# PaddlePaddle/Paddle3D

Hardware: NVIDIA H100
Metric: CenterPoint frames/sec @300k pts, 0.075m voxel (0.1m voxel: geometry_01m), 1440x1440x40 grid (higher is better)
Workload: dtype f16x3 (fp16 hi/lo' pairs, f32 accumulation)

## Files before the change

### include/p3d_b200.h

```cpp
#ifndef P3D_B200_H_
#define P3D_B200_H_

#include <stddef.h>
#include <stdint.h>

#ifdef __cplusplus
extern "C" {
#endif

typedef void *p3d_stream_t;

enum p3d_status {
  P3D_OK = 0,
  P3D_ERR_INVALID_ARG = -1,
  P3D_ERR_WORKSPACE = -2,
  P3D_ERR_CUDA = -3,
  P3D_ERR_UNSUPPORTED = -4
};

const char *p3d_status_string(int status);
int p3d_last_cuda_error(void);
int p3d_abi_version(void);

size_t p3d_hard_voxelize_workspace_bytes(int64_t num_points, int max_points, int max_voxels);
int p3d_hard_voxelize(const float *points, int64_t num_points, int num_point_dim, const float *voxel_size_host,
                      const float *point_cloud_range_host, int max_points, int max_voxels, float *voxels,
                      int32_t *coords, int32_t *num_points_per_voxel, int32_t *num_voxels, void *workspace,
                      size_t workspace_bytes, p3d_stream_t stream);

int p3d_voxelize_mean(const float *points, int64_t num_points, int num_point_dim, const float *voxel_size_host,
                      const float *point_cloud_range_host, int max_points, int max_voxels, int batch_id,
                      float *mean, int32_t *coors4, int32_t *num_points_per_voxel, int32_t *num_voxels,
                      void *workspace, size_t workspace_bytes, p3d_stream_t stream);

int p3d_voxel_mean(const float *voxels, const int32_t *num_points_per_voxel, const int32_t *num_voxels_dev,
                   int num_voxels_cap, int max_points, int num_point_dim, float *mean, p3d_stream_t stream);

size_t p3d_scatter_dense_workspace_bytes(int batch, int D, int ny, int nx);
int p3d_scatter_dense(const float *feats, const int32_t *coords, const int32_t *n_dev, int n_cap, int C,
                      int batch, int D, int ny, int nx, int use_z, float *out, void *workspace,
                      size_t workspace_bytes, p3d_stream_t stream);

int p3d_bev_pool_v2(const float *depth, const float *feat, const int32_t *ranks_depth, const int32_t *ranks_feat,
                    const int32_t *ranks_bev, const int32_t *interval_lengths, const int32_t *interval_starts,
                    int n_intervals, int c, float *out, int64_t out_numel, p3d_stream_t stream);
int p3d_bev_pool_v2_bkwd(const float *out_grad, const float *depth, const float *feat, const int32_t *ranks_depth,
                         const int32_t *ranks_feat, const int32_t *ranks_bev, const int32_t *interval_lengths,
                         const int32_t *interval_starts, int n_intervals, int c, float *depth_grad,
                         int64_t depth_numel, float *feat_grad, int64_t feat_numel, p3d_stream_t stream);

int p3d_boxes_overlap_bev(const float *boxes_a, int num_a, const float *boxes_b, int num_b, float *overlap,
                          p3d_stream_t stream);
int p3d_boxes_iou_bev(const float *boxes_a, int num_a, const float *boxes_b, int num_b, float *iou,
                      p3d_stream_t stream);
size_t p3d_nms_workspace_bytes(int n);
int p3d_nms(const float *boxes, int n, float nms_overlap_thresh, int normal, int32_t *keep, int32_t *num_keep,
            void *workspace, size_t workspace_bytes, p3d_stream_t stream);

size_t p3d_centerpoint_postprocess_workspace_bytes(int num_tasks, int feat_h, int feat_w, int nms_pre_max_size,
                                                    int nms_post_max_size);
int p3d_centerpoint_postprocess(int num_tasks, const float *const *hm, const int32_t *hm_channels_host,
                                const float *const *reg, const float *const *height, const float *const *dim,
                                const float *const *vel, const float *const *rot, int feat_h, int feat_w,
                                const float *voxel_size_host, const float *point_cloud_range_host,
                                const float *post_center_range_host, const int32_t *num_classes_host,
                                int down_ratio, float score_threshold, float nms_iou_threshold,
                                int nms_pre_max_size, int nms_post_max_size, int with_velocity, float *bboxes,
                                float *scores, int64_t *labels, int32_t *counts, void *workspace,
                                size_t workspace_bytes, p3d_stream_t stream);

size_t p3d_sparse_rulebook_workspace_bytes(int64_t n_in_cap, int64_t n_out_cap);
int p3d_sparse_rulebook_subm(const int32_t *coords, const int32_t *n_in_dev, int64_t n_in_cap, int batch,
                             const int *spatial_host, const int *ksize_host, int32_t *nbr, void *workspace,
                             size_t workspace_bytes, p3d_stream_t stream);
int p3d_sparse_rulebook_conv(const int32_t *coords, const int32_t *n_in_dev, int64_t n_in_cap, int batch,
                             const int *spatial_host, const int *ksize_host, const int *stride_host,
                             const int *pad_host, int32_t *out_coords, int32_t *n_out_dev, int64_t out_cap,
                             int32_t *nbr, void *workspace, size_t workspace_bytes, p3d_stream_t stream);

size_t p3d_sparse_table_bytes(int64_t rows_cap);
int p3d_sparse_table_build(const int32_t *coords, const int32_t *n_dev, int64_t n_cap, int batch,
                           const int *spatial_host, void *table, size_t table_bytes, p3d_stream_t stream);
int p3d_sparse_rulebook_subm_t(const int32_t *coords, const int32_t *n_dev, int64_t n_cap, int batch,
                               const int *spatial_host, const int *ksize_host, const void *table, size_t table_bytes,
                               int32_t *nbr, p3d_stream_t stream);
int p3d_sparse_rulebook_conv_t(const int32_t *coords, const int32_t *n_in_dev, int64_t n_in_cap, int batch,
                               const int *spatial_host, const int *ksize_host, const int *stride_host,
                               const int *pad_host, const void *table_in, size_t table_in_bytes, int32_t *out_coords,
                               int32_t *n_out_dev, int64_t out_cap, void *table_out, size_t table_out_bytes,
                               int32_t *nbr, p3d_stream_t stream);

int p3d_sparse_rulebook_level_t(const int32_t *coords, const int32_t *n_in_dev, int64_t n_in_cap, int batch,
                                const int *spatial_host, const int *ksize_host, const int *stride_host,
                                const int *pad_host, const void *table_in, size_t table_in_bytes, int32_t *out_coords,
                                int32_t *n_out_dev, int64_t out_cap, void *table_out, size_t table_out_bytes,
                                int32_t *nbr, const int *subm_ksize_host, int32_t *nbr_subm, p3d_stream_t stream);

int p3d_sparse_affine_act(const float *x, const int32_t *n_dev, int64_t n_cap, int C, const float *scale,
                          const float *shift, const float *residual, int relu, float *out, p3d_stream_t stream);

enum p3d_conv_precision { P3D_CONV_FP32 = 0, P3D_CONV_TF32X3 = 1 };
size_t p3d_sparse_conv_packed_weight_bytes(int K, int Cin, int Cout);
int p3d_sparse_conv_pack_weights(const float *weight, int K, int Cin, int Cout, float *packed, p3d_stream_t stream);
int p3d_sparse_conv_gather_gemm(const float *in, const int32_t *nbr, const int32_t *n_out_dev, int64_t n_out_cap,
                                int K, int Cin, int Cout, const float *weight, const float *scale,
                                const float *shift, const float *residual, int relu, int precision, float *out,
                                p3d_stream_t stream);

size_t p3d_sparse_conv_splitk_workspace_bytes(int64_t n_out_cap, int Cin, int Cout);
int p3d_sparse_conv_gather_gemm_tf32x3_ws(const float *in, const int32_t *nbr, const int32_t *n_out_dev,
                                          int64_t n_out_cap, int K, int Cin, int Cout, const float *packed_weight,
                                          const float *scale, const float *shift, const float *residual, int relu,
                                          float *out, void *workspace, size_t workspace_bytes, p3d_stream_t stream);

int p3d_rows_convert_layout(const float *src, int src_layout, const int32_t *n_dev, int64_t n_cap, int C, float *dst,
                            p3d_stream_t stream);
int p3d_sparse_conv_gather_gemm_split(const float *in_split, const int32_t *nbr, const int32_t *n_out_dev,
                                      int64_t n_out_cap, int K, int Cin, int Cout, const float *packed_weight,
                                      const float *scale, const float *shift, const float *residual_split, int relu,
                                      float *out_f32, float *out_split, p3d_stream_t stream);
int p3d_sparse_conv_gather_gemm_split_ws(const float *in_split, const int32_t *nbr, const int32_t *n_out_dev,
                                         int64_t n_out_cap, int K, int Cin, int Cout, const float *packed_weight,
                                         const float *scale, const float *shift, const float *residual_split, int relu,
                                         float *out_f32, float *out_split, void *workspace, size_t workspace_bytes,
                                         p3d_stream_t stream);
int p3d_sparse_conv_gather_gemm_split_tma(const float *in_split, int64_t n_in_rows, const int32_t *nbr,
                                          const int32_t *n_out_dev, int64_t n_out_cap, int K, int Cin, int Cout,
                                          const float *packed_weight, const float *scale, const float *shift,
                                          const float *residual_split, int relu, float *out_f32, float *out_split,
                                          void *workspace, size_t workspace_bytes, p3d_stream_t stream);

int p3d_sparse_conv_small_cin_h16(const float *in, const int32_t *nbr, const int32_t *n_out_dev, int64_t n_out_cap, int K,
                                  int Cin, int Cout, const float *weight, const float *scale, const float *shift, int relu,
                                  float *out_f32, void *out_h16, int32_t *status_dev, p3d_stream_t stream);
int p3d_sparse_rows_to_pixel_h16(const void *rows_h16, const int32_t *coords, const int32_t *n_dev, int n_cap, int C,
                                 int batch, int D, int ny, int nx, void *out_pixel_h16, p3d_stream_t stream);
size_t p3d_sparse_conv_f16_packed_weight_bytes(int K, int Cin, int Cout);
int p3d_sparse_conv_f16_pack_weights(const float *weight, int K, int Cin, int Cout, void *packed, int32_t *status_dev,
                                     p3d_stream_t stream);
int p3d_rows_convert_h16(const void *src, int to_h16, const int32_t *n_dev, int64_t n_cap, int C, void *dst,
                         int32_t *status_dev, p3d_stream_t stream);
size_t p3d_sparse_conv_f16_workspace_bytes(int64_t n_out_cap, int Cout, int max_splits);
int p3d_sparse_conv_f16(const void *in_h16, const int32_t *nbr, const int32_t *n_out_dev, int64_t n_out_cap, int K,
                        int Cin, int Cout, const void *packed_weight, const float *scale, const float *shift,
                        const void *residual_h16, int relu, float *out_f32, void *out_h16, void *workspace,
                        size_t workspace_bytes, int max_splits, int32_t *status_dev, p3d_stream_t stream);

size_t p3d_sparse_conv_wm_packed_weight_bytes(int K, int Cin, int Cout);
int p3d_sparse_conv_wm_pack_weights(const float *weight, int K, int Cin, int Cout, void *packed, int32_t *status_dev,
                                    p3d_stream_t stream);
size_t p3d_sparse_conv_wm_workspace_bytes(int64_t n_out_cap, int Cout);
int p3d_sparse_conv_wm(const void *in_h16, const int32_t *nbr, const int32_t *n_out_dev, int64_t n_out_cap, int K, int Cin,
                       int Cout, const void *packed_weight, const float *scale, const float *shift,
                       const void *residual_h16, int relu, float *out_f32, void *out_h16, void *workspace,
                       size_t workspace_bytes, int32_t *status_dev, p3d_stream_t stream);

int p3d_nchw_to_pixel_split(const float *in, int B, int C, int H, int W, float *out_split, p3d_stream_t stream);
size_t p3d_dense_conv2d_packed_weight_bytes(int taps, int Cin, int Cout, int n_tile);
int p3d_dense_conv2d_split(const float *in_split, int B, int H, int W, int Cin, const float *packed_weight, int Cout,
                           int n_tile, int kh, int kw, int stride, int pad, int up, const float *scale,
                           const float *shift, int relu, float *out_split, int out_C, int out_c0, float *out_nchw,
                           p3d_stream_t stream);

int p3d_head_final_conv(const float *in_split, int B, int H, int W, int in_C, int Cin, int groups, const float *weight,
                        const float *bias, const int32_t *plane0_host, const int32_t *cnt_host, int planes,
                        float *out_nchw, p3d_stream_t stream);
int p3d_head_final_conv_h16(const void *in_h16, int B, int H, int W, int in_C, int Cin, int groups, const float *weight,
                            const float *bias, const int32_t *plane0_host, const int32_t *cnt_host, int planes,
                            float *out_nchw, p3d_stream_t stream);

int p3d_nchw_to_pixel_h16(const float *in, int B, int C, int H, int W, void *out_h16, int32_t *status_dev,
                          p3d_stream_t stream);
int p3d_pixel_h16_to_nchw(const void *in_h16, int B, int C, int H, int W, float *out, p3d_stream_t stream);
size_t p3d_dense_conv2d_f16_packed_weight_bytes(int taps, int Cin, int Cout, int n_tile);
int p3d_dense_conv2d_f16_pack_weights(const float *weight_tci, int taps, int Cin, int n_tile, void *packed,
                                      int32_t *status_dev, p3d_stream_t stream);
size_t p3d_bev_pool_prepare_workspace_bytes(int64_t num_points);
int p3d_bev_pool_prepare(const float *coor, int B, int N, int D, int H, int W, const float *grid_lower_bound_host,
                         const float *grid_interval_host, const int32_t *grid_size_host, int32_t *ranks_bev,
                         int32_t *ranks_depth, int32_t *ranks_feat, int32_t *interval_starts, int32_t *interval_lengths,
                         int32_t *counts_dev, void *workspace, size_t workspace_bytes, p3d_stream_t stream);

int p3d_grouped_head_conv_f16(const void *in_h16, int B, int H, int W, int in_C, int Cin, int groups,
                              const void *packed_weight, const float *bias, const int32_t *plane0_dev,
                              const int32_t *cnt_dev, int planes, float *out_nchw, int32_t *status_dev, p3d_stream_t stream);
int p3d_head_out_conv_f16(const void *in_h16, int B, int H, int W, int in_C, int Cin, int groups, const void *packed_weight,
                          const float *bias, const int32_t *cin0_dev, const int32_t *plane0_dev, const int32_t *cnt_dev,
                          int planes, float *out_nchw, p3d_stream_t stream);
int p3d_dense_conv2d_f16(const void *in_h16, int B, int H, int W, int Cin, const void *packed_weight, int Cout, int n_tile,
                         int kh, int kw, int stride, int pad, int up, const float *scale, const float *shift, int relu,
                         void *out_h16, int out_C, int out_c0, float *out_nchw, int mode, int m_tiles,
                         int32_t *status_dev, p3d_stream_t stream);

int p3d_pillar_feature_net(const float *voxels, const int32_t *num_points_per_voxel, const int32_t *coors,
                           const int32_t *num_voxels_dev, int64_t n_cap, int max_points, int num_point_dim,
                           int out_channels, const float *weight, const float *bn_scale, const float *bn_shift,
                           const float *voxel_size_host, const float *point_cloud_range_host, float *out,
                           p3d_stream_t stream);

size_t p3d_anchor_head_postprocess_workspace_bytes(int num_anchors, int grid_nx, int grid_ny, int nms_pre_max_size);
int p3d_anchor_head_postprocess(const float *head, int feat_h, int feat_w, int anchors_per_loc, const float *anchors,
                                const int32_t *anchor_corners, const int32_t *coords, const int32_t *num_coords_dev,
                                int coords_cap, int grid_nx, int grid_ny, int anchor_area_threshold, float score_threshold,
                                float nms_iou_threshold, int nms_pre_max_size, int nms_post_max_size,
                                const float *post_center_range_host, float *boxes, float *scores, int64_t *labels,
                                int32_t *counts, uint8_t *anchor_mask, float *sorted_boxes, float *sorted_scores,
                                void *workspace, size_t workspace_bytes, p3d_stream_t stream);

#ifdef __cplusplus
}
#endif
#endif
```

### paddle3d_b200/_lib.py

```python
import ctypes as C
import os

_HERE = os.path.dirname(os.path.abspath(__file__))
LIB_PATH = os.path.join(_HERE, "libp3d_b200.so")
_lib = None

c_f32p = C.c_void_p
_i64 = C.c_int64
_int = C.c_int
_f = C.c_float
_sz = C.c_size_t
_vp = C.c_void_p

SIGNATURES = {
    "p3d_status_string": (C.c_char_p, [_int]),
    "p3d_last_cuda_error": (_int, []),
    "p3d_abi_version": (_int, []),
    "p3d_hard_voxelize_workspace_bytes": (_sz, [_i64, _int, _int]),
    "p3d_hard_voxelize": (_int, [_vp, _i64, _int, _vp, _vp, _int, _int, _vp, _vp, _vp, _vp, _vp, _sz, _vp]),
    "p3d_voxelize_mean": (_int, [_vp, _i64, _int, _vp, _vp, _int, _int, _int, _vp, _vp, _vp, _vp, _vp, _sz, _vp]),
    "p3d_voxel_mean": (_int, [_vp, _vp, _vp, _int, _int, _int, _vp, _vp]),
    "p3d_scatter_dense_workspace_bytes": (_sz, [_int, _int, _int, _int]),
    "p3d_scatter_dense": (_int, [_vp, _vp, _vp, _int, _int, _int, _int, _int, _int, _int, _vp, _vp, _sz, _vp]),
    "p3d_bev_pool_v2": (_int, [_vp, _vp, _vp, _vp, _vp, _vp, _vp, _int, _int, _vp, _i64, _vp]),
    "p3d_bev_pool_v2_bkwd": (_int, [_vp, _vp, _vp, _vp, _vp, _vp, _vp, _vp, _int, _int, _vp, _i64, _vp, _i64, _vp]),
    "p3d_boxes_overlap_bev": (_int, [_vp, _int, _vp, _int, _vp, _vp]),
    "p3d_boxes_iou_bev": (_int, [_vp, _int, _vp, _int, _vp, _vp]),
    "p3d_nms_workspace_bytes": (_sz, [_int]),
    "p3d_nms": (_int, [_vp, _int, _f, _int, _vp, _vp, _vp, _sz, _vp]),
    "p3d_centerpoint_postprocess_workspace_bytes": (_sz, [_int, _int, _int, _int, _int]),
    "p3d_centerpoint_postprocess": (_int, [_int, _vp, _vp, _vp, _vp, _vp, _vp, _vp, _int, _int, _vp, _vp, _vp, _vp,
                                           _int, _f, _f, _int, _int, _int, _vp, _vp, _vp, _vp, _vp, _sz, _vp]),
    "p3d_sparse_rulebook_workspace_bytes": (_sz, [_i64, _i64]),
    "p3d_sparse_rulebook_subm": (_int, [_vp, _vp, _i64, _int, _vp, _vp, _vp, _vp, _sz, _vp]),
    "p3d_sparse_rulebook_conv": (_int, [_vp, _vp, _i64, _int, _vp, _vp, _vp, _vp, _vp, _vp, _i64, _vp, _vp, _sz,
                                        _vp]),
    "p3d_sparse_table_bytes": (_sz, [_i64]),
    "p3d_sparse_table_build": (_int, [_vp, _vp, _i64, _int, _vp, _vp, _sz, _vp]),
    "p3d_sparse_rulebook_subm_t": (_int, [_vp, _vp, _i64, _int, _vp, _vp, _vp, _sz, _vp, _vp]),
    "p3d_sparse_rulebook_conv_t": (_int, [_vp, _vp, _i64, _int, _vp, _vp, _vp, _vp, _vp, _sz, _vp, _vp, _i64, _vp, _sz,
                                          _vp, _vp]),
    "p3d_sparse_rulebook_level_t": (_int, [_vp, _vp, _i64, _int, _vp, _vp, _vp, _vp, _vp, _sz, _vp, _vp, _i64, _vp, _sz,
                                           _vp, _vp, _vp, _vp]),
    "p3d_sparse_affine_act": (_int, [_vp, _vp, _i64, _int, _vp, _vp, _vp, _int, _vp, _vp]),
    "p3d_sparse_conv_packed_weight_bytes": (_sz, [_int, _int, _int]),
    "p3d_sparse_conv_pack_weights": (_int, [_vp, _int, _int, _int, _vp, _vp]),
    "p3d_rows_convert_layout": (_int, [_vp, _int, _vp, _i64, _int, _vp, _vp]),
    "p3d_sparse_conv_gather_gemm_split": (_int, [_vp, _vp, _vp, _i64, _int, _int, _int, _vp, _vp, _vp, _vp, _int, _vp,
                                                 _vp, _vp]),
    "p3d_sparse_conv_gather_gemm_split_ws": (_int, [_vp, _vp, _vp, _i64, _int, _int, _int, _vp, _vp, _vp, _vp, _int, _vp,
                                                    _vp, _vp, _sz, _vp]),
    "p3d_sparse_conv_gather_gemm_split_tma": (_int, [_vp, _i64, _vp, _vp, _i64, _int, _int, _int, _vp, _vp, _vp, _vp, _int,
                                                     _vp, _vp, _vp, _sz, _vp]),
    "p3d_sparse_conv_splitk_workspace_bytes": (_sz, [_i64, _int, _int]),
    "p3d_sparse_conv_small_cin_h16": (_int, [_vp, _vp, _vp, _i64, _int, _int, _int, _vp, _vp, _vp, _int, _vp, _vp, _vp, _vp]),
    "p3d_sparse_rows_to_pixel_h16": (_int, [_vp, _vp, _vp, _int, _int, _int, _int, _int, _int, _vp, _vp]),
    "p3d_sparse_conv_f16_packed_weight_bytes": (_sz, [_int, _int, _int]),
    "p3d_sparse_conv_f16_pack_weights": (_int, [_vp, _int, _int, _int, _vp, _vp, _vp]),
    "p3d_rows_convert_h16": (_int, [_vp, _int, _vp, _i64, _int, _vp, _vp, _vp]),
    "p3d_sparse_conv_f16_workspace_bytes": (_sz, [_i64, _int, _int]),
    "p3d_sparse_conv_f16": (_int, [_vp, _vp, _vp, _i64, _int, _int, _int, _vp, _vp, _vp, _vp, _int, _vp, _vp, _vp, _sz,
                                   _int, _vp, _vp]),
    "p3d_sparse_conv_wm_packed_weight_bytes": (_sz, [_int, _int, _int]),
    "p3d_sparse_conv_wm_pack_weights": (_int, [_vp, _int, _int, _int, _vp, _vp, _vp]),
    "p3d_sparse_conv_wm_workspace_bytes": (_sz, [_i64, _int]),
    "p3d_sparse_conv_wm": (_int, [_vp, _vp, _vp, _i64, _int, _int, _int, _vp, _vp, _vp, _vp, _int, _vp, _vp, _vp, _sz,
                                  _vp, _vp]),
    "p3d_nchw_to_pixel_split": (_int, [_vp, _int, _int, _int, _int, _vp, _vp]),
    "p3d_dense_conv2d_packed_weight_bytes": (_sz, [_int, _int, _int, _int]),
    "p3d_pillar_feature_net": (_int, [_vp, _vp, _vp, _vp, _i64, _int, _int, _int, _vp, _vp, _vp, _vp, _vp, _vp, _vp]),
    "p3d_head_final_conv": (_int, [_vp, _int, _int, _int, _int, _int, _int, _vp, _vp, _vp, _vp, _int, _vp, _vp]),
    "p3d_head_final_conv_h16": (_int, [_vp, _int, _int, _int, _int, _int, _int, _vp, _vp, _vp, _vp, _int, _vp, _vp]),
    "p3d_nchw_to_pixel_h16": (_int, [_vp, _int, _int, _int, _int, _vp, _vp, _vp]),
    "p3d_pixel_h16_to_nchw": (_int, [_vp, _int, _int, _int, _int, _vp, _vp]),
    "p3d_dense_conv2d_f16_packed_weight_bytes": (_sz, [_int, _int, _int, _int]),
    "p3d_dense_conv2d_f16_pack_weights": (_int, [_vp, _int, _int, _int, _vp, _vp, _vp]),
    "p3d_bev_pool_prepare_workspace_bytes": (_sz, [_i64]),
    "p3d_bev_pool_prepare": (_int, [_vp, _int, _int, _int, _int, _int, _vp, _vp, _vp, _vp, _vp, _vp, _vp, _vp, _vp, _vp, _sz,
                                    _vp]),
    "p3d_head_out_conv_f16": (_int, [_vp, _int, _int, _int, _int, _int, _int, _vp, _vp, _vp, _vp, _vp, _int, _vp, _vp]),
    "p3d_grouped_head_conv_f16": (_int, [_vp, _int, _int, _int, _int, _int, _int, _vp, _vp, _vp, _vp, _int, _vp, _vp, _vp]),
    "p3d_dense_conv2d_f16": (_int, [_vp, _int, _int, _int, _int, _vp, _int, _int, _int, _int, _int, _int, _int, _vp, _vp,
                                    _int, _vp, _int, _int, _vp, _int, _int, _vp, _vp]),
    "p3d_dense_conv2d_split": (_int, [_vp, _int, _int, _int, _int, _vp, _int, _int, _int, _int, _int, _int, _int, _vp, _vp,
                                      _int, _vp, _int, _int, _vp, _vp]),
    "p3d_sparse_conv_gather_gemm_tf32x3_ws": (_int, [_vp, _vp, _vp, _i64, _int, _int, _int, _vp, _vp, _vp, _vp, _int, _vp,
                                                     _vp, _sz, _vp]),
    "p3d_sparse_conv_gather_gemm": (_int, [_vp, _vp, _vp, _i64, _int, _int, _int, _vp, _vp, _vp, _vp, _int, _int,
                                           _vp, _vp]),
    "p3d_anchor_head_postprocess_workspace_bytes": (_sz, [_int, _int, _int, _int]),
    "p3d_anchor_head_postprocess": (_int, [_vp, _int, _int, _int, _vp, _vp, _vp, _vp, _int, _int, _int, _int, _f, _f,
                                           _int, _int, _vp, _vp, _vp, _vp, _vp, _vp, _vp, _vp, _vp, _sz, _vp]),
}


class P3DError(RuntimeError):
    pass


def lib():
    global _lib
    if _lib is None:
        if not os.path.exists(LIB_PATH):
            raise P3DError("libp3d_b200.so is not built: run `python -c 'import __graft_entry__ as g; g.build()'` "
                           "(paddle3d_b200 has no CPU or library fallback)")
        _lib = C.CDLL(LIB_PATH)
        for name, (res, args) in SIGNATURES.items():
            fn = getattr(_lib, name)
            fn.restype = res
            fn.argtypes = args
    return _lib


_DEBUG_SYNC = bool(os.environ.get("P3D_DEBUG_SYNC"))


def check(rc, what):
    if _DEBUG_SYNC and rc == 0:
        import torch
        try:
            torch.cuda.synchronize()
        except Exception as e:
            raise P3DError("%s: kernel fault (%s)" % (what, e))
    if rc != 0:
        l = lib()
        msg = l.p3d_status_string(rc).decode()
        extra = " (cudaError %d)" % l.p3d_last_cuda_error() if rc == -3 else ""
        raise P3DError("%s failed: %s%s" % (what, msg, extra))


def fptr(arr):
    return C.cast(arr, C.c_void_p)


def host_floats(vals):
    return (C.c_float * len(vals))(*[float(v) for v in vals])


def host_ints(vals):
    return (C.c_int * len(vals))(*[int(v) for v in vals])
```

### paddle3d_b200/csrc/dense_conv_f16.cu

```cuda
#include <cuda.h>
#include <cuda_fp16.h>

#include "p3d_b200.h"
#include "tc_common.cuh"

namespace p3d {
namespace dcf {

using namespace tc;

constexpr int kTW = 8, kTH = 16;
constexpr int kMaxA = 6, kMaxB = 12;
constexpr int kDenseThreads = 384;
constexpr uint32_t kConsumerWarps = 8;
constexpr uint32_t kEpiThreads = 96;
constexpr float kLoScale = 2048.0f, kLoInv = 1.0f / 2048.0f;

struct Params {
  int B, H, W, Cin;
  int taps, kw, stride, pad;
  int up;
  int oH, oW;
  int tiles_x, tiles_y, n_ntiles;
  int cout;
  int out_H, out_W;
  int out_C, out_c0;
  int relu;
  const uint8_t *packed_w;
  const float *scale, *shift;
  uint8_t *out_h16;
  float *out_nchw;
  int32_t *status;
  int grouped, in_C;
  const int32_t *grp_plane0, *grp_cnt;
  int base_offset_mode;
  int w_bytes;
};

template <int N, int MT, bool HALO, int PITCH, bool WS = false>
struct Cfg {
  static constexpr int A_ROWS = HALO ? PITCH * (kTH * MT + 2) : kM * MT;
  static constexpr int A_BYTES = ((A_ROWS * 128 + 1023) / 1024) * 1024;
  static constexpr int B_BYTES = 128 * N;
  static constexpr int B_BLK = 64 * N;
  static constexpr bool STAGE = !WS;
  static constexpr int SP = N + 8;
  static constexpr int STG_WG = MT * 64 * SP;
  static constexpr int STG_BYTES = STAGE ? 2 * STG_WG * 4 : 0;
  static constexpr int AVAIL = (227 - 6) * 1024 - STG_BYTES;
  static constexpr int NA_TAP_RAW = AVAIL / (A_BYTES + B_BYTES);
  static constexpr int NA = WS ? 3 : (HALO ? 2 : (NA_TAP_RAW > kMaxA ? kMaxA : NA_TAP_RAW));
  static constexpr int BUDGET = AVAIL - NA * A_BYTES;
  static constexpr int NB_RAW = BUDGET / B_BYTES;
  static constexpr int NB = NB_RAW > kMaxB ? kMaxB : NB_RAW;
  static constexpr int ACC = MT * N;
  static constexpr int SPU = HALO ? 9 : 1;
  static constexpr int P_REGS = STAGE ? 88 : 40, C_REGS = STAGE ? 208 : 232;
  static_assert(128 * P_REGS + 256 * C_REGS <= kDenseThreads * 168, "register split");
  static_assert(N == 16 || N == 64 || N == 128, "N tile: 16 (grouped output convs), 64 or 128");
  static_assert(MT == 1 || MT == 2, "one or two M tiles");
  static_assert(MT * N <= 128, "accumulators: at most 128 registers per thread");
  static_assert(WS || NB >= 3, "weight ring too shallow");
  static_assert(NA >= 2 && NA <= kMaxA, "activation ring depth");
  static_assert(!WS || (HALO && MT == 1), "weight-stationary: haloed 3x3 tiles, one M tile");
};

__device__ __forceinline__ void tma_tile4d(uint32_t dst, const CUtensorMap *map, int c, int x, int y, int b, uint32_t bar) {
  asm volatile(
      "cp.async.bulk.tensor.4d.shared::cluster.global.tile.mbarrier::complete_tx::bytes [%0], [%1, {%2, %3, %4, %5}], [%6];" ::
          "r"(dst),
      "l"(reinterpret_cast<uint64_t>(map)), "r"(c), "r"(x), "r"(y), "r"(b), "r"(bar)
      : "memory");
}
__device__ __forceinline__ void split_h16(float x, __half &hi, __half &lo, bool &ovf) {
  if (fabsf(x) > 65504.0f) {
    ovf = true;
    x = copysignf(65504.0f, x);
  }
  hi = __float2half_rn(x);
  lo = __float2half_rn((x - __half2float(hi)) * kLoScale);
}

__device__ __forceinline__ void split_h16x2(float a, float b, __half2 &hi, __half2 &lo, bool &ovf) {
  if (fabsf(a) > 65504.0f) {
    ovf = true;
    a = copysignf(65504.0f, a);
  }
  if (fabsf(b) > 65504.0f) {
    ovf = true;
    b = copysignf(65504.0f, b);
  }
  hi = __floats2half2_rn(a, b);
  const float2 h = __half22float2(hi);
  lo = __floats2half2_rn((a - h.x) * kLoScale, (b - h.y) * kLoScale);
}

struct Item {
  int nt, tap0, tx0, ty0, b;
};

enum TraceField {
  kTrItems, kTrCycles,
  kTrAFull, kTrBFull = kTrAFull + 2,
  kTrMma = kTrBFull + 2,
  kTrEpi = kTrMma + 2,
  kTrStageFree = kTrEpi + 2,
  kTrAEmpty = kTrStageFree + 2, kTrBEmpty,
  kTrEwWait, kTrEwBusy,
  kTrFields
};
#ifdef P3D_DENSE_TRACE
constexpr int kTrMaxCtas = 1024;
__device__ unsigned long long g_dense_trace[kTrMaxCtas][kTrFields];
struct Trace {
  unsigned long long sum[kTrFields] = {};
  __device__ __forceinline__ long long now() const { return clock64(); }
  __device__ __forceinline__ void add(int f, long long t0) { sum[f] += static_cast<unsigned long long>(clock64() - t0); }
  __device__ __forceinline__ void count(int f, unsigned long long v) { sum[f] += v; }
  __device__ void flush(int cw) const {
#pragma unroll
    for (int f = 0; f < kTrFields; ++f) {
      const int dst = f >= kTrAFull && f < kTrAEmpty ? f + cw : f;
      if (sum[f]) atomicAdd(&g_dense_trace[blockIdx.x % kTrMaxCtas][dst], sum[f]);
    }
  }
};
#else
struct Trace {
  __device__ __forceinline__ long long now() const { return 0; }
  __device__ __forceinline__ void add(int, long long) {}
  __device__ __forceinline__ void count(int, unsigned long long) {}
  __device__ __forceinline__ void flush(int) const {}
};
#endif
template <bool WS = false>
__device__ __forceinline__ Item decode(long long w, const Params &p, int th) {
  Item it;
  long long q = w;
  if (WS) {
    const long long pix = static_cast<long long>(p.B) * p.tiles_y * p.tiles_x;
    it.nt = static_cast<int>(q / pix);
    q -= it.nt * pix;
  } else {
    it.nt = static_cast<int>(q % p.n_ntiles);
    q /= p.n_ntiles;
  }
  it.tap0 = 0;
  if (p.up > 1) {
    const int up2 = p.up * p.up;
    it.tap0 = static_cast<int>(q % up2);
    q /= up2;
  }
  it.tx0 = static_cast<int>(q % p.tiles_x) * kTW;
  q /= p.tiles_x;
  it.ty0 = static_cast<int>(q % p.tiles_y) * th;
  it.b = static_cast<int>(q / p.tiles_y);
  return it;
}

template <int N, int MT>
__device__ __forceinline__ void epilogue_warps(const Params &p, const float *stg, unsigned long long *staged,
                                               unsigned long long *freed, long long n_items, long long w_first,
                                               long long w_step, int th, int et) {
  constexpr int SP = N + 8, ROWS = MT * 64;
  const int ew = et >> 5, lane = et & 31;
  bool ovf = false;
  Trace tr;
  for (long long idx = 0; idx < n_items; ++idx) {
    const Item im = decode<false>(w_first + idx * w_step, p, th);
    const int g_cnt = p.grouped ? __ldg(p.grp_cnt + im.nt) : 0, g_p0 = p.grouped ? __ldg(p.grp_plane0 + im.nt) : 0;
    const int dy = p.up > 1 ? im.tap0 / p.up : 0, dx = p.up > 1 ? im.tap0 % p.up : 0;
    for (int c = 0; c < 2; ++c) {
      long long t0 = tr.now();
      mbar_wait(smem_u32(staged + c), static_cast<uint32_t>(idx & 1));
      tr.add(kTrEwWait, t0);
      t0 = tr.now();
      const float *st = stg + c * ROWS * SP;
      auto pixel = [&](int r, int &Y, int &X) {
        const int m = c * 64 + (r & 63), iy = im.ty0 + (r >> 6) * kTH + m / kTW, ix = im.tx0 + m % kTW;
        Y = iy * p.up + dy;
        X = ix * p.up + dx;
        return iy < p.oH && ix < p.oW;
      };
      if (N >= 32 && p.out_h16) {
        const int r4 = lane >> 3, c4 = (lane & 7) * 4;
        for (int q = 0; q < N / 32; ++q) {
          const int col = q * 32 + c4, ch = im.nt * N + col, oc = p.out_c0 + ch;
          if (ch >= p.cout) continue;
          float sc[4], sh[4];
#pragma unroll
          for (int e = 0; e < 4; ++e) {
            sc[e] = p.scale ? __ldg(p.scale + ch + e) : 1.0f;
            sh[e] = p.shift ? __ldg(p.shift + ch + e) : 0.0f;
          }
#pragma unroll 2
          for (int rq = ew; rq < ROWS / 4; rq += 3) {
            const int r = rq * 4 + r4;
            int Y, X;
            if (!pixel(r, Y, X)) continue;
            const float4 o4 = *reinterpret_cast<const float4 *>(st + r * SP + col);
            float v[4] = {o4.x, o4.y, o4.z, o4.w};
#pragma unroll
            for (int e = 0; e < 4; ++e) {
              v[e] = fmaf(v[e], sc[e], sh[e]);
              if (p.relu) v[e] = fmaxf(v[e], 0.f);
            }
            __half2 h01, l01, h23, l23;
            split_h16x2(v[0], v[1], h01, l01, ovf);
            split_h16x2(v[2], v[3], h23, l23, ovf);
            uint8_t *op = p.out_h16 + ((static_cast<size_t>(im.b) * p.out_H + Y) * p.out_W + X) * (4 * static_cast<size_t>(p.out_C)) +
                          (oc / 32) * 128 + (oc % 32) * 2;
            *reinterpret_cast<uint2 *>(op) = make_uint2(*reinterpret_cast<const uint32_t *>(&h01), *reinterpret_cast<const uint32_t *>(&h23));
            *reinterpret_cast<uint2 *>(op + 64) = make_uint2(*reinterpret_cast<const uint32_t *>(&l01), *reinterpret_cast<const uint32_t *>(&l23));
          }
        }
      }
      if (p.out_nchw) {
        const int px = lane & 7, cc = lane >> 3;
        for (int u = ew; u < (ROWS / 8) * (N / 4); u += 3) {
          const int r = (u % (ROWS / 8)) * 8 + px, col = (u / (ROWS / 8)) * 4 + cc, ch = im.nt * N + col;
          int Y, X;
          if ((p.grouped ? col >= g_cnt : ch >= p.cout) || !pixel(r, Y, X)) continue;
          const float sc = p.scale ? __ldg(p.scale + ch) : 1.0f, sh = p.shift ? __ldg(p.shift + ch) : 0.0f;
          float v = fmaf(st[r * SP + col], sc, sh);
          if (p.relu) v = fmaxf(v, 0.f);
          const int plane = p.grouped ? g_p0 + col : ch;
          p.out_nchw[((static_cast<size_t>(im.b) * p.cout + plane) * p.out_H + Y) * p.out_W + X] = v;
        }
      }
      mbar_arrive(smem_u32(freed + c));
      tr.add(kTrEwBusy, t0);
    }
  }
  if (ovf && p.status) atomicOr(p.status, 1);
  if (et == 0) tr.flush(0);
}

template <int N, int MT, bool HALO, int PITCH, bool WS = false>
__global__ void __launch_bounds__(kDenseThreads, 1)
    dense_conv_f16_kernel(const __grid_constant__ CUtensorMap in_map, const Params p) {
  using C = Cfg<N, MT, HALO, PITCH, WS>;
  constexpr int TH = kTH * MT;
  constexpr int H = N / 2;
  asm volatile("griddepcontrol.launch_dependents;" ::: "memory");
  asm volatile("griddepcontrol.wait;" ::: "memory");
  const int up2 = p.up * p.up;
  const long long n_total = static_cast<long long>(p.B) * p.tiles_y * p.tiles_x * p.n_ntiles * (p.up > 1 ? up2 : 1);
  if (static_cast<long long>(blockIdx.x) >= n_total) return;
  const long long w_first = WS ? (static_cast<long long>(blockIdx.x) * n_total) / gridDim.x : blockIdx.x;
  const long long n_work = WS ? (static_cast<long long>(blockIdx.x + 1) * n_total) / gridDim.x : n_total;
  const long long w_step = WS ? 1 : gridDim.x;
  const long long n_items = (n_work - w_first + w_step - 1) / w_step;

  extern __shared__ __align__(1024) uint8_t smem_raw[];
  uint8_t *smem = reinterpret_cast<uint8_t *>((reinterpret_cast<uintptr_t>(smem_raw) + 1023) & ~uintptr_t(1023));
  __shared__ __align__(8) unsigned long long s_bar[2 * kMaxA + 2 * kMaxB + 6];
  constexpr int kAF = 0, kAE = kMaxA, kBF = 2 * kMaxA, kBE = 2 * kMaxA + kMaxB, kWF = 2 * kMaxA + 2 * kMaxB, kWE = kWF + 1;
  constexpr int kSS = kWE + 1, kSF = kSS + 2;

  const int tid = threadIdx.x, wg = tid >> 7, wtid = tid & 127;
  if (tid == 0) {
    for (int s = 0; s < C::NA; ++s) {
      mbar_init(smem_u32(&s_bar[kAF + s]), 1);
      mbar_init(smem_u32(&s_bar[kAE + s]), kConsumerWarps);
    }
    for (int s = 0; s < (WS ? 0 : C::NB); ++s) {
      mbar_init(smem_u32(&s_bar[kBF + s]), 1);
      mbar_init(smem_u32(&s_bar[kBE + s]), kConsumerWarps);
    }
    mbar_init(smem_u32(&s_bar[kWF]), 1);
    mbar_init(smem_u32(&s_bar[kWE]), kConsumerWarps);
    for (int c = 0; c < 2; ++c) {
      mbar_init(smem_u32(&s_bar[kSS + c]), 128);
      mbar_init(smem_u32(&s_bar[kSF + c]), kEpiThreads);
    }
    fence_mbar_init();
  }
  __syncthreads();
  const uint32_t a_ring = smem_u32(smem);
  const uint32_t b_ring = a_ring + C::NA * C::A_BYTES;
  float *const stg = reinterpret_cast<float *>(smem + C::NA * C::A_BYTES + C::NB * C::B_BYTES);
  const int G = p.Cin / 32;
  const int taps_item = p.up > 1 ? 1 : p.taps;
  const int units_item = HALO ? G : taps_item * G;
  auto item_w = [&](long long idx) { return w_first + idx * w_step; };

  if (wg == 0) {
    asm volatile("setmaxnreg.dec.sync.aligned.u32 %0;" ::"n"(C::P_REGS));
    if (tid >= 32) {
      if (C::STAGE) epilogue_warps<N, MT>(p, stg, s_bar + kSS, s_bar + kSF, n_items, w_first, w_step, TH, tid - 32);
      return;
    }
    if (tid != 0) return;
    uint32_t a_slot = 0, a_ph = 0, b_slot = 0, b_ph = 0;
    int cur_nt = -1;
    uint32_t img = 0;
    Trace tr;
    for (long long idx = 0; idx < n_items; ++idx) {
      const Item im = decode<WS>(item_w(idx), p, TH);
      const int cg0 = p.grouped ? im.nt * G : 0;
      const uint8_t *w_tile = p.packed_w + static_cast<size_t>(im.nt) * p.taps * (p.Cin / 16) * C::B_BLK;
      if (WS && im.nt != cur_nt) {
        if (img > 0) mbar_wait(smem_u32(&s_bar[kWE]), (img - 1) & 1u);
        const uint32_t bar = smem_u32(&s_bar[kWF]);
        mbar_arrive_expect_tx(bar, static_cast<uint32_t>(p.w_bytes));
        for (int off = 0; off < p.w_bytes; off += 16384) {
          const int bytes = p.w_bytes - off < 16384 ? p.w_bytes - off : 16384;
          bulk_g2s(b_ring + static_cast<uint32_t>(off), w_tile + off, static_cast<uint32_t>(bytes), bar);
        }
        ++img;
        cur_nt = im.nt;
      }
      int dy = 0, dx = 0;
      for (int tu = 0; tu < (HALO ? 1 : taps_item); ++tu) {
        const int tap = p.up > 1 ? im.tap0 : tu;
        for (int g = 0; g < G; ++g) {
          const uint32_t abar = smem_u32(&s_bar[kAF + a_slot]), a_dst = a_ring + a_slot * C::A_BYTES;
          const long long t0 = tr.now();
          mbar_wait(smem_u32(&s_bar[kAE + a_slot]), a_ph ^ 1u);
          tr.add(kTrAEmpty, t0);
          mbar_arrive_expect_tx(abar, static_cast<uint32_t>(C::A_ROWS * 128));
          if (HALO) {
            tma_tile4d(a_dst, &in_map, (cg0 + g) * 64, im.tx0 - 1, im.ty0 - 1, im.b, abar);
          } else {
            const int x = im.tx0 * p.stride - p.pad + dx, y = im.ty0 * p.stride - p.pad + dy;
            tma_tile4d(a_dst, &in_map, (cg0 + g) * 64, x, y, im.b, abar);
          }
          if (++a_slot == C::NA) a_slot = 0, a_ph ^= 1u;
          for (int t = 0; t < (WS ? 0 : C::SPU); ++t) {
            const uint32_t bbar = smem_u32(&s_bar[kBF + b_slot]);
            const long long t1 = tr.now();
            mbar_wait(smem_u32(&s_bar[kBE + b_slot]), b_ph ^ 1u);
            tr.add(kTrBEmpty, t1);
            mbar_arrive_expect_tx(bbar, static_cast<uint32_t>(C::B_BYTES));
            bulk_g2s(b_ring + b_slot * C::B_BYTES, w_tile + (static_cast<size_t>(HALO ? t : tap) * (p.Cin / 16) + 2 * g) * C::B_BLK,
                     static_cast<uint32_t>(C::B_BYTES), bbar);
            if (++b_slot == C::NB) b_slot = 0, b_ph ^= 1u;
          }
        }
        if (++dx == p.kw) dx = 0, ++dy;
      }
    }
    tr.flush(0);
    return;
  }

  asm volatile("setmaxnreg.inc.sync.aligned.u32 %0;" ::"n"(C::C_REGS));
  const int cw = wg - 1;
  const bool warp_leader = (tid & 31) == 0;
  auto release = [&](int base, uint32_t slot) {
    if (warp_leader) mbar_arrive(smem_u32(&s_bar[base + slot]));
  };
  bool ovf = false;
  uint32_t a_slot = 0, a_ph = 0, b_slot = 0, b_ph = 0;
  int cur_nt = -1;
  uint32_t img = 0;
  float acc[C::ACC];
  Trace tr;
  const long long t_start = tr.now();
  for (long long idx = 0; idx < n_items; ++idx) {
    const Item im = decode<WS>(item_w(idx), p, TH);
    if (WS && im.nt != cur_nt) {
      mbar_wait(smem_u32(&s_bar[kWF]), img & 1u);
      ++img;
      cur_nt = im.nt;
    }
#pragma unroll
    for (int i = 0; i < C::ACC; ++i) acc[i] = 0.f;
    uint32_t prev_b = 0;
    int prev_a = -1;
    bool pending = false;
    for (int ua = 0; ua < units_item; ++ua) {
      long long t0 = tr.now();
      mbar_wait(smem_u32(&s_bar[kAF + a_slot]), a_ph);
      tr.add(kTrAFull, t0);
      const uint32_t a_base = a_ring + a_slot * C::A_BYTES;
      for (int t = 0; t < C::SPU; ++t) {
        t0 = tr.now();
        if (!WS) mbar_wait(smem_u32(&s_bar[kBF + b_slot]), b_ph);
        tr.add(kTrBFull, t0);
        const uint32_t b_base = WS ? b_ring + static_cast<uint32_t>((t * (p.Cin / 16) + 2 * ua) * C::B_BLK)
                                   : b_ring + b_slot * C::B_BYTES;
        wg_fence();
#pragma unroll
        for (int kb = 0; kb < 2; ++kb) {
          const uint32_t bk = b_base + static_cast<uint32_t>(kb * C::B_BLK);
          const uint64_t dbh = smem_desc(bk, 2 * N * 16, 128), dbl = smem_desc(bk + N * 16, 2 * N * 16, 128);
#pragma unroll
          for (int mt = 0; mt < MT; ++mt) {
            uint32_t a0, sbo;
            if (HALO) {
              a0 = a_base + static_cast<uint32_t>(((mt * kTH + cw * 8 + t / 3) * PITCH + t % 3) * 128);
              sbo = PITCH * 128;
            } else {
              a0 = a_base + static_cast<uint32_t>((mt * kM + cw * 64) * 128);
              sbo = 1024;
            }
            const uint32_t ah = a0 + kb * 32, al = a0 + (2 + kb) * 32;
            const uint32_t bo = p.base_offset_mode ? 1u : 0u;
            const uint64_t dah = gmma_desc(ah, 16, sbo, 1, bo * ((ah >> 7) & 7u)), dal = gmma_desc(al, 16, sbo, 1, bo * ((al >> 7) & 7u));
            float *d = acc + mt * N;
            wg::mma_f16<N>(d, dah, dbh, 1u);
            wg::mma_f16<N>(d + H, dah, dbl, 1u);
            wg::mma_f16<N>(d + H, dal, dbh, 1u);
          }
        }
        wg_commit();
        t0 = tr.now();
        wg_wait<1>();
        tr.add(kTrMma, t0);
        if (pending) {
          if (!WS) release(kBE, prev_b);
          if (prev_a >= 0) release(kAE, static_cast<uint32_t>(prev_a));
        }
        pending = true;
        prev_b = b_slot;
        prev_a = t == C::SPU - 1 ? static_cast<int>(a_slot) : -1;
        if (!WS && ++b_slot == C::NB) b_slot = 0, b_ph ^= 1u;
      }
      if (++a_slot == C::NA) a_slot = 0, a_ph ^= 1u;
    }
    long long t0 = tr.now();
    wg_wait<0>();
    tr.add(kTrMma, t0);
    t0 = tr.now();
    if (!WS) release(kBE, prev_b);
    release(kAE, static_cast<uint32_t>(prev_a));
    if (WS && (idx + 1 == n_items || decode<WS>(item_w(idx + 1), p, TH).nt != im.nt)) release(kWE, 0);
    wg_fence_acc<C::ACC>(acc);
    if constexpr (C::STAGE) {
      tr.add(kTrEpi, t0);
      t0 = tr.now();
      if (idx > 0) mbar_wait(smem_u32(&s_bar[kSF + cw]), static_cast<uint32_t>((idx - 1) & 1));
      tr.add(kTrStageFree, t0);
      t0 = tr.now();
      float *const st = stg + cw * C::STG_WG;
#pragma unroll
      for (int mt = 0; mt < MT; ++mt) {
#pragma unroll
        for (int i = 0; i < H; i += 2) {
          const int r = mt * 64 + frag_row(i, wtid), c = frag_col(i, wtid);
          *reinterpret_cast<float2 *>(st + r * C::SP + c) =
              make_float2(fmaf(acc[mt * N + H + i], kLoInv, acc[mt * N + i]), fmaf(acc[mt * N + H + i + 1], kLoInv, acc[mt * N + i + 1]));
        }
      }
      mbar_arrive(smem_u32(&s_bar[kSS + cw]));
      tr.add(kTrEpi, t0);
      continue;
    }

    const int g_cnt = p.grouped ? __ldg(p.grp_cnt + im.nt) : 0, g_p0 = p.grouped ? __ldg(p.grp_plane0 + im.nt) : 0;
#pragma unroll
    for (int mt = 0; mt < MT; ++mt) {
#pragma unroll
      for (int i = 0; i < H; i += 2) {
        const int m = cw * 64 + frag_row(i, wtid), c = frag_col(i, wtid);
        const int iy = im.ty0 + mt * kTH + m / kTW, ix = im.tx0 + m % kTW;
        const int ch = im.nt * N + c;
        if (iy >= p.oH || ix >= p.oW || (p.grouped ? c >= g_cnt : ch >= p.cout)) continue;
        const int Y = iy * p.up + (p.up > 1 ? im.tap0 / p.up : 0), X = ix * p.up + (p.up > 1 ? im.tap0 % p.up : 0);
        const size_t opix = (static_cast<size_t>(im.b) * p.out_H + Y) * p.out_W + X;
        float v[2];
#pragma unroll
        for (int e = 0; e < 2; ++e) {
          const bool okc = p.grouped ? true : ch + e < p.cout;
          const float sc = (p.scale && okc) ? __ldg(p.scale + ch + e) : 1.0f, sh = (p.shift && okc) ? __ldg(p.shift + ch + e) : 0.0f;
          float o = fmaf(acc[mt * N + H + i + e], kLoInv, acc[mt * N + i + e]);
          o = fmaf(o, sc, sh);
          if (p.relu) o = fmaxf(o, 0.f);
          v[e] = o;
        }
        if (p.out_h16) {
          __half h0, l0, h1, l1;
          split_h16(v[0], h0, l0, ovf);
          split_h16(v[1], h1, l1, ovf);
          const int oc = p.out_c0 + ch;
          uint8_t *op = p.out_h16 + opix * (4 * static_cast<size_t>(p.out_C)) + (oc / 32) * 128 + (oc % 32) * 2;
          *reinterpret_cast<__half2 *>(op) = __halves2half2(h0, h1);
          *reinterpret_cast<__half2 *>(op + 64) = __halves2half2(l0, l1);
        }
        if (p.out_nchw) {
#pragma unroll
          for (int e = 0; e < 2; ++e) {
            if (p.grouped) {
              if (c + e < g_cnt) p.out_nchw[((static_cast<size_t>(im.b) * p.cout + g_p0 + c + e) * p.out_H + Y) * p.out_W + X] = v[e];
            } else if (ch + e < p.cout) {
              p.out_nchw[((static_cast<size_t>(im.b) * p.cout + ch + e) * p.out_H + Y) * p.out_W + X] = v[e];
            }
          }
        }
      }
    }
    tr.add(kTrEpi, t0);
  }
  if (ovf && p.status) atomicOr(p.status, 1);
  if (cw == 0) {
    tr.count(kTrItems, static_cast<unsigned long long>(n_items));
    tr.add(kTrCycles, t_start);
  }
  if (wtid == 0) tr.flush(cw);
}

__global__ void __launch_bounds__(256) nchw_to_pixel_h16_kernel(const float *__restrict__ in, int C, long long HW,
                                                                __half *__restrict__ out, int32_t *status) {
  __shared__ float s_t[32][33];
  const int b = blockIdx.z;
  const long long p0 = static_cast<long long>(blockIdx.x) * 32;
  const int c0 = blockIdx.y * 32;
  const int tx = threadIdx.x & 31, ty = threadIdx.x >> 5;
  for (int k = ty; k < 32; k += 8) {
    const int c = c0 + k;
    const long long px = p0 + tx;
    s_t[k][tx] = (c < C && px < HW) ? in[(static_cast<size_t>(b) * C + c) * HW + px] : 0.f;
  }
  __syncthreads();
  bool ovf = false;
  for (int k = ty; k < 32; k += 8) {
    const long long px = p0 + k;
    if (px < HW) {
      __half h, l;
      split_h16(s_t[tx][k], h, l, ovf);
      __half *grp = out + (static_cast<size_t>(b) * HW + px) * (2 * static_cast<size_t>(C)) + static_cast<size_t>(c0) * 2;
      grp[tx] = h;
      grp[32 + tx] = l;
    }
  }
  if (ovf && status) atomicOr(status, 1);
}

__global__ void __launch_bounds__(256) pixel_h16_to_nchw_kernel(const __half *__restrict__ in, int C, long long HW,
                                                                float *__restrict__ out, long long total) {
  const long long q = static_cast<long long>(blockIdx.x) * blockDim.x + threadIdx.x;
  if (q >= total) return;
  const long long px = q % HW;
  const int c = static_cast<int>((q / HW) % C);
  const long long b = q / (HW * C);
  const __half *grp = in + (b * HW + px) * (2 * static_cast<long long>(C)) + (c / 32) * 64;
  out[q] = fmaf(__half2float(grp[32 + c % 32]), kLoInv, __half2float(grp[c % 32]));
}

inline int make_image_map(const void *img, int B, int H, int W, int Cin, int stride, int box_x, int box_y, CUtensorMap *map) {
  using Encode = CUresult (*)(CUtensorMap *, CUtensorMapDataType, cuuint32_t, void *, const cuuint64_t *, const cuuint64_t *,
                              const cuuint32_t *, const cuuint32_t *, CUtensorMapInterleave, CUtensorMapSwizzle,
                              CUtensorMapL2promotion, CUtensorMapFloatOOBfill);
  static Encode encode = nullptr;
  if (!encode) {
    void *fn = nullptr;
    cudaDriverEntryPointQueryResult qr;
    if (cudaGetDriverEntryPoint("cuTensorMapEncodeTiled", &fn, cudaEnableDefault, &qr) != cudaSuccess || !fn)
      return P3D_ERR_UNSUPPORTED;
    encode = reinterpret_cast<Encode>(fn);
  }
  const cuuint64_t row = static_cast<cuuint64_t>(4) * Cin;
  const cuuint64_t gdim[4] = {static_cast<cuuint64_t>(2 * Cin), static_cast<cuuint64_t>(W), static_cast<cuuint64_t>(H),
                              static_cast<cuuint64_t>(B)};
  const cuuint64_t gstride[3] = {row, row * W, row * W * H};
  const cuuint32_t box[4] = {64u, static_cast<cuuint32_t>(box_x * stride), static_cast<cuuint32_t>(box_y * stride), 1u};
  const cuuint32_t estride[4] = {1u, static_cast<cuuint32_t>(stride), static_cast<cuuint32_t>(stride), 1u};
  const CUresult r = encode(map, CU_TENSOR_MAP_DATA_TYPE_FLOAT16, 4, const_cast<void *>(img), gdim, gstride, box, estride,
                            CU_TENSOR_MAP_INTERLEAVE_NONE, CU_TENSOR_MAP_SWIZZLE_128B, CU_TENSOR_MAP_L2_PROMOTION_NONE,
                            CU_TENSOR_MAP_FLOAT_OOB_FILL_NONE);
  return r == CUDA_SUCCESS ? P3D_OK : P3D_ERR_INVALID_ARG;
}

template <int N, int MT, bool HALO, int PITCH, bool WS = false>
int launch(const CUtensorMap &map, const Params &p, cudaStream_t st) {
  using C = Cfg<N, MT, HALO, PITCH, WS>;
  const size_t smem = static_cast<size_t>(C::NA) * C::A_BYTES +
                      (WS ? static_cast<size_t>(p.w_bytes) : static_cast<size_t>(C::NB) * C::B_BYTES) + C::STG_BYTES + 1024;
  if (smem > static_cast<size_t>(227 - 6) * 1024) return P3D_ERR_UNSUPPORTED;
  auto kern = dense_conv_f16_kernel<N, MT, HALO, PITCH, WS>;
  P3D_CUDA_CHECK(cudaFuncSetAttribute(kern, cudaFuncAttributeMaxDynamicSharedMemorySize, static_cast<int>(smem)));
  const long long work = static_cast<long long>(p.B) * p.tiles_y * p.tiles_x * p.n_ntiles * (p.up > 1 ? p.up * p.up : 1);
  cudaLaunchConfig_t cfg = {};
  const long long sms = num_sms();
  cfg.gridDim = dim3(static_cast<unsigned int>(work < sms ? work : sms));
  cfg.blockDim = dim3(kDenseThreads);
  cfg.dynamicSmemBytes = smem;
  cfg.stream = st;
  cudaLaunchAttribute attr[1];
  attr[0].id = cudaLaunchAttributeProgrammaticStreamSerialization;
  attr[0].val.programmaticStreamSerializationAllowed = 1;
  cfg.attrs = attr;
  cfg.numAttrs = 1;
  P3D_CUDA_CHECK(cudaLaunchKernelEx(&cfg, kern, map, p));
  P3D_LAUNCH_CHECK();
  return P3D_OK;
}

namespace out9 {
constexpr int kHT = 16, kOT = 14;
constexpr int kRows = kHT * kHT;
constexpr int kABytes = kRows * 128;
constexpr int kN = 32, kStride = 29;
constexpr int kWBlk = 64 * kN;
constexpr int kPBytes = kRows * kStride * 4;
constexpr int kMaxNA = 5, kNW = 3;
constexpr int kAcc = 2 * kN;

struct Params {
  int B, H, W, G;
  int tiles_x, tiles_y, groups, planes, NA;
  const uint8_t *packed_w;
  const float *bias;
  const int32_t *cin0;
  const int32_t *plane0, *cnt;
  float *out;
};

__global__ void __launch_bounds__(kThreads, 1) head_out9_kernel(const __grid_constant__ CUtensorMap in_map, const Params p) {
  asm volatile("griddepcontrol.launch_dependents;" ::: "memory");
  asm volatile("griddepcontrol.wait;" ::: "memory");
  const long long n_work = static_cast<long long>(p.B) * p.tiles_y * p.tiles_x * p.groups;
  if (static_cast<long long>(blockIdx.x) >= n_work) return;
  extern __shared__ __align__(1024) uint8_t smem_raw[];
  uint8_t *smem = reinterpret_cast<uint8_t *>((reinterpret_cast<uintptr_t>(smem_raw) + 1023) & ~uintptr_t(1023));
  __shared__ __align__(8) unsigned long long s_bar[kMaxNA + kNW];
  constexpr int kAF = 0, kWF = kMaxNA;
  const int tid = threadIdx.x, wg = tid >> 7, wtid = tid & 127;
  const int NA = p.NA, G = p.G;
  const uint32_t w_slot = static_cast<uint32_t>(2 * G * kWBlk);
  if (tid == 0) {
    for (int s = 0; s < NA; ++s) mbar_init(smem_u32(&s_bar[kAF + s]), 1);
    for (int s = 0; s < kNW; ++s) mbar_init(smem_u32(&s_bar[kWF + s]), 1);
    fence_mbar_init();
  }
  const uint32_t a_ring = smem_u32(smem);
  const uint32_t w_ring = a_ring + static_cast<uint32_t>(NA * kABytes);
  float *s_p = reinterpret_cast<float *>(smem + static_cast<size_t>(NA) * kABytes + static_cast<size_t>(kNW) * w_slot);

  auto decode = [&](long long w, int &g, int &tx0, int &ty0, int &b) {
    g = static_cast<int>(w % p.groups);
    long long q = w / p.groups;
    tx0 = static_cast<int>(q % p.tiles_x) * kOT;
    q /= p.tiles_x;
    ty0 = static_cast<int>(q % p.tiles_y) * kOT;
    b = static_cast<int>(q / p.tiles_y);
  };
  const long long n_items = (n_work - blockIdx.x + gridDim.x - 1) / gridDim.x;
  const long long n_steps = n_items * G;
  auto issue_a = [&](long long q) {
    int g, tx0, ty0, b;
    decode(blockIdx.x + (q / G) * gridDim.x, g, tx0, ty0, b);
    const int cg0 = (p.cin0 ? __ldg(p.cin0 + g) : g * G * 32) / 32;
    const uint32_t slot = static_cast<uint32_t>(q % NA), bar = smem_u32(&s_bar[kAF + slot]);
    mbar_arrive_expect_tx(bar, static_cast<uint32_t>(kABytes));
    tma_tile4d(a_ring + slot * kABytes, &in_map, (cg0 + static_cast<int>(q % G)) * 64, tx0 - 1, ty0 - 1, b, bar);
  };
  auto issue_w = [&](long long i) {
    const int g = static_cast<int>((blockIdx.x + i * gridDim.x) % p.groups);
    const uint32_t slot = static_cast<uint32_t>(i % kNW), bar = smem_u32(&s_bar[kWF + slot]);
    mbar_arrive_expect_tx(bar, w_slot);
    bulk_g2s(w_ring + slot * w_slot, p.packed_w + static_cast<size_t>(g) * w_slot, w_slot, bar);
  };

  long long next_a = 0, next_w = 0, q = 0;
  float acc[kAcc];
  for (long long idx = 0; idx < n_items; ++idx) {
    int g, tx0, ty0, b;
    decode(blockIdx.x + idx * gridDim.x, g, tx0, ty0, b);
    const int cnt = __ldg(p.cnt + g), p0 = __ldg(p.plane0 + g);
    const float4 bias = __ldg(reinterpret_cast<const float4 *>(p.bias) + g);
#pragma unroll
    for (int i = 0; i < kAcc; ++i) acc[i] = 0.f;
    const uint32_t ws = static_cast<uint32_t>(idx % kNW);
    for (int k = 0; k < G; ++k, ++q) {
      __syncthreads();
      if (tid == 0) {
        for (; next_a < n_steps && next_a <= q + NA - 1; ++next_a) issue_a(next_a);
        for (; next_w < n_items && (next_w - kNW + 1) * G <= q; ++next_w) issue_w(next_w);
      }
      if (k == 0) mbar_wait(smem_u32(&s_bar[kWF + ws]), static_cast<uint32_t>((idx / kNW) & 1));
      const uint32_t sa = static_cast<uint32_t>(q % NA);
      mbar_wait(smem_u32(&s_bar[kAF + sa]), static_cast<uint32_t>((q / NA) & 1));
      const uint32_t a_base = a_ring + sa * kABytes;
      const uint32_t w_base = w_ring + ws * w_slot;
      wg_fence();
#pragma unroll
      for (int kb = 0; kb < 2; ++kb) {
        const uint32_t bk = w_base + static_cast<uint32_t>((k * 2 + kb) * kWBlk);
        const uint64_t dbh = smem_desc(bk, 2 * kN * 16, 128), dbl = smem_desc(bk + kN * 16, 2 * kN * 16, 128);
#pragma unroll
        for (int mt = 0; mt < 2; ++mt) {
          const uint32_t a0 = a_base + static_cast<uint32_t>((mt * kM + wg * 64) * 128);
          const uint64_t dah = desc_sw128(a0 + kb * 32), dal = desc_sw128(a0 + (2 + kb) * 32);
          float *d = acc + mt * kN;
          wg::mma_f16<kN>(d, dah, dbh, 1u);
          wg::mma_f16<kN>(d + kN / 2, dah, dbl, 1u);
          wg::mma_f16<kN>(d + kN / 2, dal, dbh, 1u);
        }
      }
      wg_commit();
      wg_wait<0>();
    }
    wg_fence_acc<kAcc>(acc);
#pragma unroll
    for (int mt = 0; mt < 2; ++mt) {
#pragma unroll
      for (int i = 0; i < kN / 2; ++i) {
        const int r = mt * kM + wg * 64 + frag_row(i, wtid), c = frag_col(i, wtid);
        if (c < 27) s_p[r * kStride + c] = fmaf(acc[mt * kN + kN / 2 + i], kLoInv, acc[mt * kN + i]);
      }
    }
    __syncthreads();
    for (int o = tid; o < kOT * kOT; o += kThreads) {
      const int oy = o / kOT, ox = o - oy * kOT;
      const int Y = ty0 + oy, X = tx0 + ox;
      if (Y < p.H && X < p.W) {
        float s0 = bias.x, s1 = bias.y, s2 = bias.z;
#pragma unroll
        for (int t = 0; t < 9; ++t) {
          const float *e = s_p + ((oy + t / 3) * kHT + ox + t % 3) * kStride + t * 3;
          s0 += e[0];
          s1 += e[1];
          s2 += e[2];
        }
        float *op = p.out + ((static_cast<size_t>(b) * p.planes + p0) * p.H + Y) * p.W + X;
        const size_t plane = static_cast<size_t>(p.H) * p.W;
        op[0] = s0;
        if (cnt > 1) op[plane] = s1;
        if (cnt > 2) op[2 * plane] = s2;
      }
    }
  }
}
}

}
}

using namespace p3d;

extern "C" int p3d_nchw_to_pixel_h16(const float *in, int B, int C, int H, int W, void *out_h16, int32_t *status_dev,
                                     p3d_stream_t stream) {
  if (!in || !out_h16 || B < 1 || C < 32 || C % 32 || H < 1 || W < 1) return P3D_ERR_INVALID_ARG;
  const long long hw = static_cast<long long>(H) * W;
  dim3 grid(static_cast<unsigned int>((hw + 31) / 32), static_cast<unsigned int>(C / 32), B);
  dcf::nchw_to_pixel_h16_kernel<<<grid, 256, 0, static_cast<cudaStream_t>(stream)>>>(in, C, hw, static_cast<__half *>(out_h16),
                                                                                      status_dev);
  P3D_LAUNCH_CHECK();
  return P3D_OK;
}

extern "C" int p3d_pixel_h16_to_nchw(const void *in_h16, int B, int C, int H, int W, float *out, p3d_stream_t stream) {
  if (!in_h16 || !out || B < 1 || C < 32 || C % 32 || H < 1 || W < 1) return P3D_ERR_INVALID_ARG;
  const long long hw = static_cast<long long>(H) * W, total = hw * C * B;
  dcf::pixel_h16_to_nchw_kernel<<<div_up(total, 256), 256, 0, static_cast<cudaStream_t>(stream)>>>(
      static_cast<const __half *>(in_h16), C, hw, out, total);
  P3D_LAUNCH_CHECK();
  return P3D_OK;
}

#ifdef P3D_DENSE_TRACE
extern "C" int p3d_dense_trace_read(unsigned long long *host, int max_ctas, int reset) {
  const size_t n = static_cast<size_t>(max_ctas < dcf::kTrMaxCtas ? max_ctas : dcf::kTrMaxCtas) * dcf::kTrFields;
  P3D_CUDA_CHECK(cudaDeviceSynchronize());
  if (host) P3D_CUDA_CHECK(cudaMemcpyFromSymbol(host, dcf::g_dense_trace, n * sizeof(unsigned long long)));
  if (reset) {
    void *dev = nullptr;
    P3D_CUDA_CHECK(cudaGetSymbolAddress(&dev, dcf::g_dense_trace));
    P3D_CUDA_CHECK(cudaMemset(dev, 0, sizeof(dcf::g_dense_trace)));
    P3D_CUDA_CHECK(cudaDeviceSynchronize());
  }
  return dcf::kTrFields;
}
#endif

extern "C" size_t p3d_dense_conv2d_f16_packed_weight_bytes(int taps, int Cin, int Cout, int n_tile) {
  if (taps < 1 || Cin < 32 || Cin % 32 || Cout < 1 || (n_tile != 16 && n_tile != 32 && n_tile != 64 && n_tile != 128)) return 0;
  const size_t tiles = static_cast<size_t>((Cout + n_tile - 1) / n_tile);
  return align_up(tiles * taps * Cin * static_cast<size_t>(n_tile) * 4);
}

static int dense_conv_f16(const void *in_h16, int B, int H, int W, int Cin, const void *packed_weight, int Cout, int n_tile,
                          int kh, int kw, int stride, int pad, int up, const float *scale, const float *shift, int relu,
                          void *out_h16, int out_C, int out_c0, float *out_nchw, int mode, int m_tiles, int32_t *status_dev,
                          p3d_stream_t stream, int groups, int in_C, const int32_t *grp_plane0, const int32_t *grp_cnt) {
  if (!in_h16 || !packed_weight || (!out_h16 && !out_nchw) || B < 1 || H < 1 || W < 1 || Cout < 1) return P3D_ERR_INVALID_ARG;
  if (Cin < 32 || Cin % 32 || (n_tile != 64 && n_tile != 128 && !(groups && n_tile == 16))) return P3D_ERR_UNSUPPORTED;
  if (up < 1 || (up > 1 && (kh != up || kw != up || stride != up || pad != 0))) return P3D_ERR_UNSUPPORTED;
  if (up == 1 && (kh < 1 || kw < 1 || kh * kw > 32 || stride < 1 || stride > 2 || pad < 0)) return P3D_ERR_UNSUPPORTED;
  if (out_h16 && (Cout % 16 || out_C % 32 || out_c0 % 16 || out_c0 + Cout > out_C)) return P3D_ERR_INVALID_ARG;
  if ((reinterpret_cast<uintptr_t>(in_h16) & 15) || (reinterpret_cast<uintptr_t>(packed_weight) & 15) ||
      (reinterpret_cast<uintptr_t>(out_h16) & 15))
    return P3D_ERR_INVALID_ARG;
  dcf::Params p;
  p.B = B;
  p.H = H;
  p.W = W;
  p.Cin = Cin;
  p.taps = kh * kw;
  p.kw = kw;
  p.up = up;
  p.stride = up > 1 ? 1 : stride;
  p.pad = up > 1 ? 0 : pad;
  p.oH = up > 1 ? H : (H + 2 * pad - kh) / stride + 1;
  p.oW = up > 1 ? W : (W + 2 * pad - kw) / stride + 1;
  if (p.oH < 1 || p.oW < 1) return P3D_ERR_INVALID_ARG;
  p.out_H = up > 1 ? H * up : p.oH;
  p.out_W = up > 1 ? W * up : p.oW;
  p.n_ntiles = groups ? groups : (Cout + n_tile - 1) / n_tile;
  p.cout = Cout;
  p.grouped = groups ? 1 : 0;
  p.in_C = groups ? in_C : Cin;
  p.grp_plane0 = grp_plane0;
  p.grp_cnt = grp_cnt;
  p.out_C = out_C;
  p.out_c0 = out_c0;
  p.relu = relu;
  p.packed_w = static_cast<const uint8_t *>(packed_weight);
  p.scale = scale;
  p.shift = shift;
  p.out_h16 = static_cast<uint8_t *>(out_h16);
  p.out_nchw = out_nchw;
  p.status = status_dev;
  static const int env_mode = getenv("P3D_DENSE_MODE") ? atoi(getenv("P3D_DENSE_MODE")) : -1;
  static const int env_mt = getenv("P3D_DENSE_MT") ? atoi(getenv("P3D_DENSE_MT")) : -1;
  static const int env_pitch = getenv("P3D_DENSE_PITCH") ? atoi(getenv("P3D_DENSE_PITCH")) : 10;
  static const int env_bo = getenv("P3D_DENSE_BO") ? atoi(getenv("P3D_DENSE_BO")) : 0;
  p.base_offset_mode = env_bo;
  int pitch = env_pitch == 16 ? 16 : 10;
  if (env_mode >= 0) mode = env_mode;
  if (env_mt >= 0) m_tiles = env_mt;
  const bool halo = (mode == 0 || mode == 2) && up == 1 && kh == 3 && kw == 3 && stride == 1 && pad == 1;
  int mt = m_tiles;
  if (mt != 1 && mt != 2) {
    const long long tx = (p.oW + dcf::kTW - 1) / dcf::kTW, sms = num_sms();
    const long long per_row = static_cast<long long>(B) * tx * p.n_ntiles * (up > 1 ? up * up : 1);
    const long long items1 = per_row * ((p.oH + dcf::kTH - 1) / dcf::kTH), items2 = per_row * ((p.oH + 2 * dcf::kTH - 1) / (2 * dcf::kTH));
    mt = (n_tile <= 64 && 2 * ((items2 + sms - 1) / sms) <= (items1 + sms - 1) / sms) ? 2 : 1;
  }
  static const int env_ws = getenv("P3D_DENSE_WS") ? atoi(getenv("P3D_DENSE_WS")) : 0;
  p.w_bytes = p.taps * (Cin / 16) * 64 * n_tile;
  bool ws = false;
  if (halo && n_tile == 64 && !groups && pitch == 10 && (env_ws || mode == 2)) {
    const size_t need = 3 * static_cast<size_t>(dcf::Cfg<64, 1, true, 10, true>::A_BYTES) + p.w_bytes + 1024;
    const long long pix = static_cast<long long>(B) * ((p.oW + dcf::kTW - 1) / dcf::kTW) * ((p.oH + dcf::kTH - 1) / dcf::kTH);
    const long long items = pix * p.n_ntiles;
    ws = need <= static_cast<size_t>(227 - 6) * 1024 && (mode == 2 || items >= 8ll * num_sms());
  }
  if (mode == 2 && !ws) return P3D_ERR_UNSUPPORTED;
  if (ws || n_tile > 64) mt = 1;
  if (mt == 2) pitch = 10;
  p.tiles_x = (p.oW + dcf::kTW - 1) / dcf::kTW;
  p.tiles_y = (p.oH + dcf::kTH * mt - 1) / (dcf::kTH * mt);
  CUtensorMap map;
  const int bx = halo ? pitch : dcf::kTW, by = halo ? dcf::kTH * mt + 2 : dcf::kTH * mt;
  const int rc = dcf::make_image_map(in_h16, B, H, W, p.in_C, p.stride, bx, by, &map);
  if (rc != P3D_OK) return rc;
  cudaStream_t st = static_cast<cudaStream_t>(stream);
  if (ws) return dcf::launch<64, 1, true, 10, true>(map, p, st);
#define P3D_DCF(NT, M)                                                                          \
  if (n_tile == NT && mt == M) {                                                                \
    if (!halo) return dcf::launch<NT, M, false, 10>(map, p, st);                                \
    if (M == 1 && pitch == 16) return dcf::launch<NT, 1, true, 16>(map, p, st);                 \
    return dcf::launch<NT, M, true, 10>(map, p, st);                                            \
  }
  P3D_DCF(16, 1)
  P3D_DCF(16, 2)
  P3D_DCF(64, 1)
  P3D_DCF(64, 2)
  P3D_DCF(128, 1)
#undef P3D_DCF
  return P3D_ERR_UNSUPPORTED;
}

extern "C" int p3d_dense_conv2d_f16(const void *in_h16, int B, int H, int W, int Cin, const void *packed_weight, int Cout,
                                    int n_tile, int kh, int kw, int stride, int pad, int up, const float *scale,
                                    const float *shift, int relu, void *out_h16, int out_C, int out_c0, float *out_nchw,
                                    int mode, int m_tiles, int32_t *status_dev, p3d_stream_t stream) {
  return dense_conv_f16(in_h16, B, H, W, Cin, packed_weight, Cout, n_tile, kh, kw, stride, pad, up, scale, shift, relu, out_h16,
                        out_C, out_c0, out_nchw, mode, m_tiles, status_dev, stream, 0, 0, nullptr, nullptr);
}

extern "C" int p3d_grouped_head_conv_f16(const void *in_h16, int B, int H, int W, int in_C, int Cin, int groups,
                                         const void *packed_weight, const float *bias, const int32_t *plane0_dev,
                                         const int32_t *cnt_dev, int planes, float *out_nchw, int32_t *status_dev,
                                         p3d_stream_t stream) {
  if (!plane0_dev || !cnt_dev || groups < 1 || groups * Cin > in_C || in_C % 32 || planes < 1) return P3D_ERR_INVALID_ARG;
  return dense_conv_f16(in_h16, B, H, W, Cin, packed_weight, planes, 16, 3, 3, 1, 1, 1, nullptr, bias, 0, nullptr, 32, 0, out_nchw,
                        0, 0, status_dev, stream, groups, in_C, plane0_dev, cnt_dev);
}

extern "C" int p3d_head_out_conv_f16(const void *in_h16, int B, int H, int W, int in_C, int Cin, int groups,
                                     const void *packed_weight, const float *bias, const int32_t *cin0_dev,
                                     const int32_t *plane0_dev, const int32_t *cnt_dev, int planes, float *out_nchw,
                                     p3d_stream_t stream) {
  if (!in_h16 || !packed_weight || !bias || !plane0_dev || !cnt_dev || !out_nchw || B < 1 || H < 1 || W < 1 || groups < 1 ||
      planes < 1 || in_C % 32 || Cin > in_C)
    return P3D_ERR_INVALID_ARG;
  if (Cin != 32 && Cin != 64 && Cin != 128) return P3D_ERR_UNSUPPORTED;
  if ((reinterpret_cast<uintptr_t>(in_h16) & 15) || (reinterpret_cast<uintptr_t>(packed_weight) & 15) ||
      (reinterpret_cast<uintptr_t>(bias) & 15))
    return P3D_ERR_INVALID_ARG;
  namespace o9 = dcf::out9;
  o9::Params p;
  p.B = B;
  p.H = H;
  p.W = W;
  p.G = Cin / 32;
  p.tiles_x = (W + o9::kOT - 1) / o9::kOT;
  p.tiles_y = (H + o9::kOT - 1) / o9::kOT;
  p.groups = groups;
  p.planes = planes;
  p.NA = p.G <= 2 ? 5 : 4;
  p.packed_w = static_cast<const uint8_t *>(packed_weight);
  p.bias = bias;
  p.cin0 = cin0_dev;
  p.plane0 = plane0_dev;
  p.cnt = cnt_dev;
  p.out = out_nchw;
  CUtensorMap map;
  const int rc = dcf::make_image_map(in_h16, B, H, W, in_C, 1, o9::kHT, o9::kHT, &map);
  if (rc != P3D_OK) return rc;
  const size_t smem = static_cast<size_t>(p.NA) * o9::kABytes + static_cast<size_t>(o9::kNW) * 2 * p.G * o9::kWBlk + o9::kPBytes + 1024;
  auto kern = o9::head_out9_kernel;
  P3D_CUDA_CHECK(cudaFuncSetAttribute(kern, cudaFuncAttributeMaxDynamicSharedMemorySize, static_cast<int>(smem)));
  const long long work = static_cast<long long>(B) * p.tiles_y * p.tiles_x * groups;
  cudaLaunchConfig_t cfg = {};
  const long long sms = num_sms();
  cfg.gridDim = dim3(static_cast<unsigned int>(work < sms ? work : sms));
  cfg.blockDim = dim3(tc::kThreads);
  cfg.dynamicSmemBytes = smem;
  cfg.stream = static_cast<cudaStream_t>(stream);
  cudaLaunchAttribute attr[1];
  attr[0].id = cudaLaunchAttributeProgrammaticStreamSerialization;
  attr[0].val.programmaticStreamSerializationAllowed = 1;
  cfg.attrs = attr;
  cfg.numAttrs = 1;
  P3D_CUDA_CHECK(cudaLaunchKernelEx(&cfg, kern, map, p));
  P3D_LAUNCH_CHECK();
  return P3D_OK;
}
```

### paddle3d_b200/ops/dense_conv.py

```python
import torch

from .._lib import check, lib
from .._mem import ptr, require_cuda, stream


def n_tile_for(cout):
    return 128 if cout >= 128 else (64 if cout > 16 else 16)


def nchw_to_pixel_split(x):
    x = require_cuda(x, "x", torch.float32)
    b, c, h, w = x.shape
    out = torch.empty((b * h * w, 2 * c), dtype=torch.float32, device=x.device)
    check(lib().p3d_nchw_to_pixel_split(ptr(x), b, c, h, w, ptr(out), stream(x.device)), "nchw_to_pixel_split")
    return out


def _pack(w_tci, n_tile):
    L = lib()
    taps, cin, cout = w_tci.shape
    tiles = (cout + n_tile - 1) // n_tile
    total = L.p3d_dense_conv2d_packed_weight_bytes(taps, cin, cout, n_tile)
    if not total:
        raise ValueError("unsupported dense conv shape: taps %d Cin %d Cout %d" % (taps, cin, cout))
    packed = torch.zeros((total // 4,), dtype=torch.float32, device=w_tci.device)
    padded = torch.zeros((taps, cin, tiles * n_tile), dtype=torch.float32, device=w_tci.device)
    padded[:, :, :cout] = w_tci
    block = taps * cin * 2 * n_tile
    for t in range(tiles):
        wt = padded[:, :, t * n_tile:(t + 1) * n_tile].contiguous()
        dst = packed[t * block:(t + 1) * block]
        check(L.p3d_sparse_conv_pack_weights(ptr(wt), taps, cin, n_tile, ptr(dst), stream(wt.device)),
              "sparse_conv_pack_weights")
    return packed


def pack_conv_weight(weight, n_tile):
    weight = require_cuda(weight, "weight", torch.float32)
    cout, cin, kh, kw = weight.shape
    return _pack(weight.permute(2, 3, 1, 0).reshape(kh * kw, cin, cout).contiguous(), n_tile)


def pack_deconv_weight(weight, n_tile):
    weight = require_cuda(weight, "weight", torch.float32)
    cin, cout, k, k2 = weight.shape
    return _pack(weight.permute(2, 3, 0, 1).reshape(k * k2, cin, cout).contiguous(), n_tile)


def dense_conv2d(x_split, shape, packed, cout, n_tile, kernel, stride=1, padding=0, up=1, scale=None, shift=None,
                 relu=False, out_split=None, out_channels=None, out_c0=0, want_nchw=False):
    x_split = require_cuda(x_split, "x_split", torch.float32)
    b, h, w, cin = [int(v) for v in shape]
    if up > 1:
        oh, ow = h * up, w * up
        kh = kw = st = up
        pd = 0
    else:
        kh = kw = int(kernel)
        st, pd = int(stride), int(padding)
        oh, ow = (h + 2 * pd - kh) // st + 1, (w + 2 * pd - kw) // st + 1
    dev = x_split.device
    oc = int(out_channels or cout)
    if out_split is None and not want_nchw:
        out_split = torch.empty((b * oh * ow, 2 * oc), dtype=torch.float32, device=dev)
    out_nchw = torch.empty((b, cout, oh, ow), dtype=torch.float32, device=dev) if want_nchw else None
    check(lib().p3d_dense_conv2d_split(ptr(x_split), b, h, w, cin, ptr(packed), int(cout), int(n_tile), kh, kw, st, pd,
                                       int(up), ptr(scale), ptr(shift), int(relu), ptr(out_split), oc, int(out_c0),
                                       ptr(out_nchw), stream(dev)), "dense_conv2d_split")
    return out_split, out_nchw, (b, oh, ow)


def n_tile_for_f16(cout, cin=None, kernel=None, stride=1, padding=0, up=1):
    import os
    forced = os.environ.get("P3D_DENSE_NTILE")
    if forced and cout >= 128:
        return int(forced)
    if (cin is not None and kernel == 3 and stride == 1 and padding == 1 and up == 1 and cin <= 64 and cout >= 256
            and os.environ.get("P3D_DENSE_WS", "0") != "0"):
        return 64
    return 128 if cout >= 128 else 64


def _status(dev):
    from . import sparse_nn as sp
    return sp.status_tensor(dev)


def nchw_to_pixel_h16(x):
    x = require_cuda(x, "x", torch.float32)
    b, c, h, w = x.shape
    out = torch.empty((b * h * w, 2 * c), dtype=torch.float16, device=x.device)
    check(lib().p3d_nchw_to_pixel_h16(ptr(x), b, c, h, w, ptr(out), ptr(_status(x.device)), stream(x.device)),
          "nchw_to_pixel_h16")
    return out


def pixel_h16_to_nchw(x_h16, shape):
    b, h, w, c = [int(v) for v in shape]
    out = torch.empty((b, c, h, w), dtype=torch.float32, device=x_h16.device)
    check(lib().p3d_pixel_h16_to_nchw(ptr(x_h16), b, c, h, w, ptr(out), stream(x_h16.device)), "pixel_h16_to_nchw")
    return out


def _pack_f16(w_tci, n_tile):
    L = lib()
    taps, cin, cout = w_tci.shape
    tiles = (cout + n_tile - 1) // n_tile
    total = L.p3d_dense_conv2d_f16_packed_weight_bytes(taps, cin, cout, n_tile)
    if not total:
        raise ValueError("unsupported dense conv shape: taps %d Cin %d Cout %d" % (taps, cin, cout))
    packed = torch.zeros((total,), dtype=torch.uint8, device=w_tci.device)
    padded = torch.zeros((taps, cin, tiles * n_tile), dtype=torch.float32, device=w_tci.device)
    padded[:, :, :cout] = w_tci
    block = taps * cin * n_tile * 4
    for t in range(tiles):
        wt = padded[:, :, t * n_tile:(t + 1) * n_tile].contiguous()
        dst = packed[t * block:(t + 1) * block]
        check(L.p3d_dense_conv2d_f16_pack_weights(ptr(wt), taps, cin, n_tile, ptr(dst), ptr(_status(wt.device)),
                                                  stream(wt.device)), "dense_conv2d_f16_pack_weights")
    return packed


def pack_conv_weight_f16(weight, n_tile):
    weight = require_cuda(weight, "weight", torch.float32)
    cout, cin, kh, kw = weight.shape
    return _pack_f16(weight.permute(2, 3, 1, 0).reshape(kh * kw, cin, cout).contiguous(), n_tile)


def pack_deconv_weight_f16(weight, n_tile):
    weight = require_cuda(weight, "weight", torch.float32)
    cin, cout, k, k2 = weight.shape
    return _pack_f16(weight.permute(2, 3, 0, 1).reshape(k * k2, cin, cout).contiguous(), n_tile)


def dense_conv2d_f16(x_h16, shape, packed, cout, n_tile, kernel, stride=1, padding=0, up=1, scale=None, shift=None,
                     relu=False, out_h16=None, out_channels=None, out_c0=0, want_nchw=False, mode=0, m_tiles=0):
    x_h16 = require_cuda(x_h16, "x_h16", torch.float16)
    b, h, w, cin = [int(v) for v in shape]
    if up > 1:
        oh, ow = h * up, w * up
        kh = kw = st = up
        pd = 0
    else:
        kh = kw = int(kernel)
        st, pd = int(stride), int(padding)
        oh, ow = (h + 2 * pd - kh) // st + 1, (w + 2 * pd - kw) // st + 1
    dev = x_h16.device
    oc = int(out_channels or cout)
    if out_h16 is None and not want_nchw:
        out_h16 = torch.empty((b * oh * ow, 2 * oc), dtype=torch.float16, device=dev)
    out_nchw = torch.empty((b, cout, oh, ow), dtype=torch.float32, device=dev) if want_nchw else None
    check(lib().p3d_dense_conv2d_f16(ptr(x_h16), b, h, w, cin, ptr(packed), int(cout), int(n_tile), kh, kw, st, pd, int(up),
                                     ptr(scale), ptr(shift), int(relu), ptr(out_h16), oc, int(out_c0), ptr(out_nchw),
                                     int(mode), int(m_tiles), ptr(_status(dev)), stream(dev)), "dense_conv2d_f16")
    return out_h16, out_nchw, (b, oh, ow)
```

### paddle_ext/p3d_paddle_ops.cc

```cpp
#include <vector>

#include "paddle/extension.h"
#include "p3d_b200.h"

#define P3D_CHECK_GPU(x) PD_CHECK((x).is_gpu() || (x).is_gpu_pinned(), #x " must be a GPU Tensor.")
#define P3D_CALL(expr)                                                                 \
  do {                                                                                 \
    int _rc = (expr);                                                                  \
    if (_rc != 0) PD_THROW(std::string(#expr " failed: ") + p3d_status_string(_rc)); \
  } while (0)

namespace {

paddle::Tensor workspace(size_t bytes) {
  return paddle::empty({static_cast<int64_t>(bytes ? bytes : 256)}, paddle::DataType::UINT8, paddle::GPUPlace());
}

}

std::vector<paddle::Tensor> hard_voxelize(const paddle::Tensor &points, const std::vector<float> &voxel_size,
                                          const std::vector<float> &point_cloud_range,
                                          const int max_num_points_in_voxel, const int max_voxels) {
  P3D_CHECK_GPU(points);
  const int64_t n = points.shape()[0];
  const int f = static_cast<int>(points.shape()[1]);
  auto voxels = paddle::empty({max_voxels, max_num_points_in_voxel, f}, paddle::DataType::FLOAT32, paddle::GPUPlace());
  auto coords = paddle::empty({max_voxels, 3}, paddle::DataType::INT32, paddle::GPUPlace());
  auto npv = paddle::empty({max_voxels}, paddle::DataType::INT32, paddle::GPUPlace());
  auto num_voxels = paddle::empty({1}, paddle::DataType::INT32, paddle::GPUPlace());
  const size_t ws_bytes = p3d_hard_voxelize_workspace_bytes(n, max_num_points_in_voxel, max_voxels);
  auto ws = workspace(ws_bytes);
  P3D_CALL(p3d_hard_voxelize(points.data<float>(), n, f, voxel_size.data(), point_cloud_range.data(),
                             max_num_points_in_voxel, max_voxels, voxels.data<float>(), coords.data<int>(),
                             npv.data<int>(), num_voxels.data<int>(), ws.data<uint8_t>(), ws_bytes, points.stream()));
  return {voxels, coords, npv, num_voxels};
}

std::vector<std::vector<int64_t>> HardInferShape(std::vector<int64_t> points_shape, const std::vector<float> &voxel_size,
                                                 const std::vector<float> &point_cloud_range,
                                                 const int &max_num_points_in_voxel, const int &max_voxels) {
  return {{max_voxels, max_num_points_in_voxel, points_shape[1]}, {max_voxels, 3}, {max_voxels}, {1}};
}

std::vector<paddle::DataType> HardInferDtype(paddle::DataType points_dtype) {
  return {points_dtype, paddle::DataType::INT32, paddle::DataType::INT32, paddle::DataType::INT32};
}

PD_BUILD_OP(hard_voxelize)
    .Inputs({"POINTS"})
    .Outputs({"VOXELS", "COORS", "NUM_POINTS_PER_VOXEL", "num_voxels"})
    .SetKernelFn(PD_KERNEL(hard_voxelize))
    .Attrs({"voxel_size: std::vector<float>", "point_cloud_range: std::vector<float>", "max_num_points_in_voxel: int",
            "max_voxels: int"})
    .SetInferShapeFn(PD_INFER_SHAPE(HardInferShape))
    .SetInferDtypeFn(PD_INFER_DTYPE(HardInferDtype));

static std::vector<paddle::Tensor> pairwise(const paddle::Tensor &a, const paddle::Tensor &b, bool iou) {
  P3D_CHECK_GPU(a);
  P3D_CHECK_GPU(b);
  const int na = static_cast<int>(a.shape()[0]), nb = static_cast<int>(b.shape()[0]);
  auto out = paddle::empty({na, nb}, paddle::DataType::FLOAT32, paddle::GPUPlace());
  if (iou)
    P3D_CALL(p3d_boxes_iou_bev(a.data<float>(), na, b.data<float>(), nb, out.data<float>(), a.stream()));
  else
    P3D_CALL(p3d_boxes_overlap_bev(a.data<float>(), na, b.data<float>(), nb, out.data<float>(), a.stream()));
  return {out};
}
std::vector<paddle::Tensor> boxes_iou_bev_gpu(const paddle::Tensor &a, const paddle::Tensor &b) { return pairwise(a, b, true); }
std::vector<paddle::Tensor> boxes_overlap_bev_gpu(const paddle::Tensor &a, const paddle::Tensor &b) {
  return pairwise(a, b, false);
}

static std::vector<paddle::Tensor> nms_any(const paddle::Tensor &boxes, float thresh, int normal) {
  P3D_CHECK_GPU(boxes);
  const int n = static_cast<int>(boxes.shape()[0]);
  auto keep_dev = paddle::empty({n > 0 ? n : 1}, paddle::DataType::INT32, paddle::GPUPlace());
  auto num_dev = paddle::empty({1}, paddle::DataType::INT32, paddle::GPUPlace());
  const size_t ws_bytes = p3d_nms_workspace_bytes(n);
  auto ws = workspace(ws_bytes);
  P3D_CALL(p3d_nms(boxes.data<float>(), n, thresh, normal, keep_dev.data<int>(), num_dev.data<int>(),
                   ws.data<uint8_t>(), ws_bytes, boxes.stream()));
  return {keep_dev.copy_to(paddle::CPUPlace(), true), num_dev.copy_to(paddle::CPUPlace(), true)};
}
std::vector<paddle::Tensor> nms_gpu(const paddle::Tensor &boxes, float nms_overlap_thresh) {
  return nms_any(boxes, nms_overlap_thresh, 0);
}
std::vector<paddle::Tensor> nms_normal_gpu(const paddle::Tensor &boxes, float nms_overlap_thresh) {
  return nms_any(boxes, nms_overlap_thresh, 1);
}

std::vector<paddle::DataType> PairInferDtype(paddle::DataType a, paddle::DataType b) { return {a}; }
std::vector<std::vector<int64_t>> PairInferShape(std::vector<int64_t> a, std::vector<int64_t> b) { return {{a[0], b[0]}}; }
std::vector<paddle::DataType> NmsInferDtype(paddle::DataType boxes_dtype) {
  return {paddle::DataType::INT64, paddle::DataType::INT64};
}
std::vector<std::vector<int64_t>> NmsInferShape(std::vector<int64_t> boxes_shape) { return {{boxes_shape[0]}, {1}}; }

PD_BUILD_OP(boxes_iou_bev_gpu)
    .Inputs({"boxes_a_tensor", " boxes_b_tensor"})
    .Outputs({"ans_iou_tensor"})
    .SetKernelFn(PD_KERNEL(boxes_iou_bev_gpu))
    .SetInferDtypeFn(PD_INFER_DTYPE(PairInferDtype))
    .SetInferShapeFn(PD_INFER_SHAPE(PairInferShape));
PD_BUILD_OP(boxes_overlap_bev_gpu)
    .Inputs({"boxes_a", " boxes_b"})
    .Outputs({"ans_overlap"})
    .SetKernelFn(PD_KERNEL(boxes_overlap_bev_gpu))
    .SetInferDtypeFn(PD_INFER_DTYPE(PairInferDtype))
    .SetInferShapeFn(PD_INFER_SHAPE(PairInferShape));
PD_BUILD_OP(nms_gpu)
    .Inputs({"boxes"})
    .Outputs({"keep", "num_to_keep"})
    .Attrs({"nms_overlap_thresh: float"})
    .SetKernelFn(PD_KERNEL(nms_gpu))
    .SetInferDtypeFn(PD_INFER_DTYPE(NmsInferDtype))
    .SetInferShapeFn(PD_INFER_SHAPE(NmsInferShape));
PD_BUILD_OP(nms_normal_gpu)
    .Inputs({"boxes"})
    .Outputs({"keep", "num_to_keep"})
    .Attrs({"nms_overlap_thresh: float"})
    .SetKernelFn(PD_KERNEL(nms_normal_gpu))
    .SetInferDtypeFn(PD_INFER_DTYPE(NmsInferDtype))
    .SetInferShapeFn(PD_INFER_SHAPE(NmsInferShape));

std::vector<paddle::Tensor> centerpoint_postprocess(
    const std::vector<paddle::Tensor> &hm, const std::vector<paddle::Tensor> &reg,
    const std::vector<paddle::Tensor> &height, const std::vector<paddle::Tensor> &dim,
    const std::vector<paddle::Tensor> &vel, const std::vector<paddle::Tensor> &rot, const std::vector<float> &voxel_size,
    const std::vector<float> &point_cloud_range, const std::vector<float> &post_center_range,
    const std::vector<int> &num_classes, const int down_ratio, const float score_threshold,
    const float nms_iou_threshold, const int nms_pre_max_size, const int nms_post_max_size, const bool with_velocity) {
  if (!hm[0].is_gpu()) PD_THROW("Unsupported device type for centerpoint postprocess operator.");
  PD_CHECK(hm[0].shape()[0] == 1, "hm[0] batch size must be 1.");
  const int T = static_cast<int>(hm.size());
  const int H = static_cast<int>(hm[0].shape()[2]), W = static_cast<int>(hm[0].shape()[3]);
  std::vector<const float *> p[6];
  std::vector<int32_t> hm_c(T);
  const std::vector<paddle::Tensor> *lists[6] = {&hm, &reg, &height, &dim, &vel, &rot};
  for (int k = 0; k < 6; ++k)
    for (int t = 0; t < T; ++t) p[k].push_back((*lists[k])[t].data<float>());
  for (int t = 0; t < T; ++t) hm_c[t] = static_cast<int32_t>(hm[t].shape()[1]);
  const int dims = with_velocity ? 9 : 7;
  const int rows = T * (nms_post_max_size > 1 ? nms_post_max_size : 1);
  auto bboxes = paddle::empty({rows, dims}, paddle::DataType::FLOAT32, paddle::GPUPlace());
  auto scores = paddle::empty({rows}, paddle::DataType::FLOAT32, paddle::GPUPlace());
  auto labels = paddle::empty({rows}, paddle::DataType::INT64, paddle::GPUPlace());
  auto counts = paddle::empty({T + 1}, paddle::DataType::INT32, paddle::GPUPlace());
  const size_t ws_bytes = p3d_centerpoint_postprocess_workspace_bytes(T, H, W, nms_pre_max_size, nms_post_max_size);
  auto ws = workspace(ws_bytes);
  P3D_CALL(p3d_centerpoint_postprocess(T, p[0].data(), hm_c.data(), p[1].data(), p[2].data(), p[3].data(), p[4].data(),
                                       p[5].data(), H, W, voxel_size.data(), point_cloud_range.data(),
                                       post_center_range.data(), num_classes.data(), down_ratio, score_threshold,
                                       nms_iou_threshold, nms_pre_max_size, nms_post_max_size, with_velocity ? 1 : 0,
                                       bboxes.data<float>(), scores.data<float>(), labels.data<int64_t>(),
                                       counts.data<int>(), ws.data<uint8_t>(), ws_bytes, hm[0].stream()));
  const int k = counts.copy_to(paddle::CPUPlace(), true).data<int>()[T];
  return {paddle::experimental::slice(bboxes, {0}, {0}, {k}, {}, {}), paddle::experimental::slice(scores, {0}, {0}, {k}, {}, {}),
          paddle::experimental::slice(labels, {0}, {0}, {k}, {}, {})};
}

std::vector<std::vector<int64_t>> PostProcessInferShape(
    const std::vector<std::vector<int64_t>> &hm_shape, const std::vector<std::vector<int64_t>> &reg_shape,
    const std::vector<std::vector<int64_t>> &height_shape, const std::vector<std::vector<int64_t>> &dim_shape,
    const std::vector<std::vector<int64_t>> &vel_shape, const std::vector<std::vector<int64_t>> &rot_shape,
    const std::vector<float> &voxel_size, const std::vector<float> &point_cloud_range,
    const std::vector<float> &post_center_range, const std::vector<int> &num_classes, const int down_ratio,
    const float score_threshold, const float nms_iou_threshold, const int nms_pre_max_size,
    const int nms_post_max_size, const bool with_velocity) {
  if (with_velocity) return {{-1, 9}, {-1}, {-1}};
  return {{-1, 7}, {-1}, {-1}};
}

std::vector<paddle::DataType> PostProcessInferDtype(
    const std::vector<paddle::DataType> &hm_dtype, const std::vector<paddle::DataType> &reg_dtype,
    const std::vector<paddle::DataType> &height_dtype, const std::vector<paddle::DataType> &dim_dtype,
    const std::vector<paddle::DataType> &vel_dtype, const std::vector<paddle::DataType> &rot_dtype) {
  return {reg_dtype[0], hm_dtype[0], paddle::DataType::INT64};
}

PD_BUILD_OP(centerpoint_postprocess)
    .Inputs({paddle::Vec("HM"), paddle::Vec("REG"), paddle::Vec("HEIGHT"), paddle::Vec("DIM"), paddle::Vec("VEL"),
             paddle::Vec("ROT")})
    .Outputs({"BBOXES", "SCORES", "LABELS"})
    .SetKernelFn(PD_KERNEL(centerpoint_postprocess))
    .Attrs({"voxel_size: std::vector<float>", "point_cloud_range: std::vector<float>",
            "post_center_range: std::vector<float>", "num_classes: std::vector<int>", "down_ratio: int",
            "score_threshold: float", "nms_iou_threshold: float", "nms_pre_max_size: int", "nms_post_max_size: int",
            "with_velocity: bool"})
    .SetInferShapeFn(PD_INFER_SHAPE(PostProcessInferShape))
    .SetInferDtypeFn(PD_INFER_DTYPE(PostProcessInferDtype));

std::vector<paddle::Tensor> bev_pool_v2_forward(const paddle::Tensor &_depth, const paddle::Tensor &_feat,
                                                const paddle::Tensor &_ranks_depth, const paddle::Tensor &_ranks_feat,
                                                const paddle::Tensor &_ranks_bev, const paddle::Tensor &_interval_lengths,
                                                const paddle::Tensor &_interval_starts,
                                                const std::vector<int> &_bev_feat_shape) {
  P3D_CHECK_GPU(_feat);
  const int c = static_cast<int>(_feat.shape()[3]);
  const int n_intervals = static_cast<int>(_interval_lengths.shape()[0]);
  std::vector<int64_t> shape(_bev_feat_shape.begin(), _bev_feat_shape.end());
  auto out = paddle::empty(shape, _feat.type(), paddle::GPUPlace());
  P3D_CALL(p3d_bev_pool_v2(_depth.data<float>(), _feat.data<float>(), _ranks_depth.data<int>(), _ranks_feat.data<int>(),
                           _ranks_bev.data<int>(), _interval_lengths.data<int>(), _interval_starts.data<int>(),
                           n_intervals, c, out.data<float>(), out.numel(), _feat.stream()));
  return {out};
}

std::vector<paddle::Tensor> bev_pool_v2_backward(const paddle::Tensor &_out_grad, const paddle::Tensor &_depth,
                                                 const paddle::Tensor &_feat, const paddle::Tensor &_ranks_depth,
                                                 const paddle::Tensor &_ranks_feat, const paddle::Tensor &_ranks_bev,
                                                 const paddle::Tensor &_interval_lengths,
                                                 const paddle::Tensor &_interval_starts) {
  P3D_CHECK_GPU(_out_grad);
  const int c = static_cast<int>(_out_grad.shape()[3]);
  const int n_intervals = static_cast<int>(_interval_lengths.shape()[0]);
  auto depth_grad = paddle::empty(_depth.shape(), _depth.type(), paddle::GPUPlace());
  auto feat_grad = paddle::empty(_feat.shape(), _feat.type(), paddle::GPUPlace());
  P3D_CALL(p3d_bev_pool_v2_bkwd(_out_grad.data<float>(), _depth.data<float>(), _feat.data<float>(),
                                _ranks_depth.data<int>(), _ranks_feat.data<int>(), _ranks_bev.data<int>(),
                                _interval_lengths.data<int>(), _interval_starts.data<int>(), n_intervals, c,
                                depth_grad.data<float>(), depth_grad.numel(), feat_grad.data<float>(), feat_grad.numel(),
                                _out_grad.stream()));
  return {depth_grad, feat_grad};
}

std::vector<std::vector<int64_t>> BevPoolV2InferShape(std::vector<int64_t> a, std::vector<int64_t> b, std::vector<int64_t> c,
                                                      std::vector<int64_t> d, std::vector<int64_t> e, std::vector<int64_t> f,
                                                      std::vector<int64_t> g, const std::vector<int> _bev_feat_shape) {
  return {{_bev_feat_shape[0], _bev_feat_shape[1], _bev_feat_shape[2], _bev_feat_shape[3]}};
}
std::vector<paddle::DataType> BevPoolV2InferDtype(paddle::DataType a, paddle::DataType feat, paddle::DataType c,
                                                  paddle::DataType d, paddle::DataType e, paddle::DataType f,
                                                  paddle::DataType g) {
  return {feat};
}

PD_BUILD_OP(bev_pool_v2)
    .Inputs({"_depth", "_feat", "_ranks_depth", "_ranks_feat", "_ranks_bev", "_interval_lengths", "_interval_starts"})
    .Attrs({"_bev_feat_shape: std::vector<int>"})
    .Outputs({"out"})
    .SetKernelFn(PD_KERNEL(bev_pool_v2_forward))
    .SetInferShapeFn(PD_INFER_SHAPE(BevPoolV2InferShape))
    .SetInferDtypeFn(PD_INFER_DTYPE(BevPoolV2InferDtype));

std::vector<std::vector<int64_t>> BevPoolV2BkwdInferShape(std::vector<int64_t> og, std::vector<int64_t> depth,
                                                          std::vector<int64_t> feat, std::vector<int64_t> d,
                                                          std::vector<int64_t> e, std::vector<int64_t> f,
                                                          std::vector<int64_t> g, std::vector<int64_t> h) {
  return {depth, feat};
}
std::vector<paddle::DataType> BevPoolV2BkwdInferDtype(paddle::DataType og, paddle::DataType depth, paddle::DataType feat,
                                                      paddle::DataType d, paddle::DataType e, paddle::DataType f,
                                                      paddle::DataType g, paddle::DataType h) {
  return {depth, feat};
}

PD_BUILD_OP(bev_pool_v2_bkwd)
    .Inputs({"_out_grad", "_depth", "_feat", "_ranks_depth", "_ranks_feat", "_ranks_bev", "_interval_lengths",
             "_interval_starts"})
    .Outputs({"_depth_grad", "_feat_grad"})
    .SetKernelFn(PD_KERNEL(bev_pool_v2_backward))
    .SetInferShapeFn(PD_INFER_SHAPE(BevPoolV2BkwdInferShape))
    .SetInferDtypeFn(PD_INFER_DTYPE(BevPoolV2BkwdInferDtype));


std::vector<paddle::Tensor> p3d_scatter_dense_op(const paddle::Tensor &feats, const paddle::Tensor &coords,
                                                 const paddle::Tensor &num, const int batch, const int D, const int ny,
                                                 const int nx, const int use_z) {
  P3D_CHECK_GPU(feats);
  const int n = static_cast<int>(feats.shape()[0]), C = static_cast<int>(feats.shape()[1]);
  auto out = paddle::empty({batch, static_cast<int64_t>(C) * D, ny, nx}, paddle::DataType::FLOAT32, paddle::GPUPlace());
  const size_t ws_bytes = p3d_scatter_dense_workspace_bytes(batch, D, ny, nx);
  auto ws = workspace(ws_bytes);
  P3D_CALL(p3d_scatter_dense(feats.data<float>(), coords.data<int>(), num.data<int>(), n, C, batch, D, ny, nx, use_z,
                             out.data<float>(), ws.data<uint8_t>(), ws_bytes, feats.stream()));
  return {out};
}
std::vector<std::vector<int64_t>> ScatterInferShape(std::vector<int64_t> f, std::vector<int64_t> c, std::vector<int64_t> n,
                                                    const int &batch, const int &D, const int &ny, const int &nx,
                                                    const int &use_z) {
  return {{batch, f[1] * D, ny, nx}};
}
std::vector<paddle::DataType> ScatterInferDtype(paddle::DataType f, paddle::DataType c, paddle::DataType n) { return {f}; }

PD_BUILD_OP(p3d_scatter_dense)
    .Inputs({"FEATS", "COORDS", "NUM"})
    .Outputs({"OUT"})
    .Attrs({"batch: int", "D: int", "ny: int", "nx: int", "use_z: int"})
    .SetKernelFn(PD_KERNEL(p3d_scatter_dense_op))
    .SetInferShapeFn(PD_INFER_SHAPE(ScatterInferShape))
    .SetInferDtypeFn(PD_INFER_DTYPE(ScatterInferDtype));

std::vector<paddle::Tensor> p3d_subm_rulebook_op(const paddle::Tensor &coords, const paddle::Tensor &num, const int batch,
                                                 const std::vector<int> &spatial, const std::vector<int> &ksize) {
  P3D_CHECK_GPU(coords);
  const int64_t cap = coords.shape()[0];
  const int64_t K = static_cast<int64_t>(ksize[0]) * ksize[1] * ksize[2];
  auto nbr = paddle::empty({cap, K}, paddle::DataType::INT32, paddle::GPUPlace());
  const size_t ws_bytes = p3d_sparse_rulebook_workspace_bytes(cap, cap);
  auto ws = workspace(ws_bytes);
  P3D_CALL(p3d_sparse_rulebook_subm(coords.data<int>(), num.data<int>(), cap, batch, spatial.data(), ksize.data(),
                                    nbr.data<int>(), ws.data<uint8_t>(), ws_bytes, coords.stream()));
  return {nbr};
}
std::vector<std::vector<int64_t>> SubmRbInferShape(std::vector<int64_t> c, std::vector<int64_t> n, const int &batch,
                                                   const std::vector<int> &spatial, const std::vector<int> &ksize) {
  return {{c[0], static_cast<int64_t>(ksize[0]) * ksize[1] * ksize[2]}};
}
std::vector<paddle::DataType> SubmRbInferDtype(paddle::DataType c, paddle::DataType n) { return {paddle::DataType::INT32}; }

PD_BUILD_OP(p3d_sparse_subm_rulebook)
    .Inputs({"COORDS", "NUM"})
    .Outputs({"NBR"})
    .Attrs({"batch: int", "spatial: std::vector<int>", "ksize: std::vector<int>"})
    .SetKernelFn(PD_KERNEL(p3d_subm_rulebook_op))
    .SetInferShapeFn(PD_INFER_SHAPE(SubmRbInferShape))
    .SetInferDtypeFn(PD_INFER_DTYPE(SubmRbInferDtype));

std::vector<paddle::Tensor> p3d_conv_rulebook_op(const paddle::Tensor &coords, const paddle::Tensor &num, const int batch,
                                                 const std::vector<int> &spatial, const std::vector<int> &ksize,
                                                 const std::vector<int> &stride, const std::vector<int> &padding,
                                                 const int out_cap) {
  P3D_CHECK_GPU(coords);
  const int64_t cap = coords.shape()[0];
  const int64_t K = static_cast<int64_t>(ksize[0]) * ksize[1] * ksize[2];
  auto out_coords = paddle::empty({out_cap, 4}, paddle::DataType::INT32, paddle::GPUPlace());
  auto n_out = paddle::empty({4}, paddle::DataType::INT32, paddle::GPUPlace());
  auto nbr = paddle::empty({out_cap, K}, paddle::DataType::INT32, paddle::GPUPlace());
  const size_t ws_bytes = p3d_sparse_rulebook_workspace_bytes(cap, out_cap);
  auto ws = workspace(ws_bytes);
  P3D_CALL(p3d_sparse_rulebook_conv(coords.data<int>(), num.data<int>(), cap, batch, spatial.data(), ksize.data(),
                                    stride.data(), padding.data(), out_coords.data<int>(), n_out.data<int>(), out_cap,
                                    nbr.data<int>(), ws.data<uint8_t>(), ws_bytes, coords.stream()));
  return {out_coords, n_out, nbr};
}
std::vector<std::vector<int64_t>> ConvRbInferShape(std::vector<int64_t> c, std::vector<int64_t> n, const int &batch,
                                                   const std::vector<int> &spatial, const std::vector<int> &ksize,
                                                   const std::vector<int> &stride, const std::vector<int> &padding,
                                                   const int &out_cap) {
  return {{out_cap, 4}, {4}, {out_cap, static_cast<int64_t>(ksize[0]) * ksize[1] * ksize[2]}};
}
std::vector<paddle::DataType> ConvRbInferDtype(paddle::DataType c, paddle::DataType n) {
  return {paddle::DataType::INT32, paddle::DataType::INT32, paddle::DataType::INT32};
}

PD_BUILD_OP(p3d_sparse_conv_rulebook)
    .Inputs({"COORDS", "NUM"})
    .Outputs({"OUT_COORDS", "OUT_NUM", "NBR"})
    .Attrs({"batch: int", "spatial: std::vector<int>", "ksize: std::vector<int>", "stride: std::vector<int>",
            "padding: std::vector<int>", "out_cap: int"})
    .SetKernelFn(PD_KERNEL(p3d_conv_rulebook_op))
    .SetInferShapeFn(PD_INFER_SHAPE(ConvRbInferShape))
    .SetInferDtypeFn(PD_INFER_DTYPE(ConvRbInferDtype));

std::vector<paddle::Tensor> p3d_gather_gemm_op(const paddle::Tensor &in, const paddle::Tensor &nbr, const paddle::Tensor &num,
                                               const paddle::Tensor &weight, const paddle::Tensor &scale,
                                               const paddle::Tensor &shift, const paddle::Tensor &residual, const int relu,
                                               const int precision) {
  P3D_CHECK_GPU(in);
  const int64_t cap = nbr.shape()[0];
  const int K = static_cast<int>(nbr.shape()[1]);
  const int Cin = static_cast<int>(in.shape()[1]);
  const int Cout = static_cast<int>(weight.shape()[weight.shape().size() - 1]);
  auto out = paddle::empty({cap, Cout}, paddle::DataType::FLOAT32, paddle::GPUPlace());
  const float *res = residual.numel() > 1 ? residual.data<float>() : nullptr;
  P3D_CALL(p3d_sparse_conv_gather_gemm(in.data<float>(), nbr.data<int>(), num.data<int>(), cap, K, Cin, Cout,
                                       weight.data<float>(), scale.data<float>(), shift.data<float>(), res, relu,
                                       precision, out.data<float>(), in.stream()));
  return {out};
}
std::vector<std::vector<int64_t>> GgInferShape(std::vector<int64_t> in, std::vector<int64_t> nbr, std::vector<int64_t> num,
                                               std::vector<int64_t> w, std::vector<int64_t> sc, std::vector<int64_t> sh,
                                               std::vector<int64_t> res, const int &relu, const int &precision) {
  return {{nbr[0], w[w.size() - 1]}};
}
std::vector<paddle::DataType> GgInferDtype(paddle::DataType in, paddle::DataType nbr, paddle::DataType num, paddle::DataType w,
                                           paddle::DataType sc, paddle::DataType sh, paddle::DataType res) {
  return {in};
}

PD_BUILD_OP(p3d_sparse_gather_gemm)
    .Inputs({"IN", "NBR", "NUM", "WEIGHT", "SCALE", "SHIFT", "RESIDUAL"})
    .Outputs({"OUT"})
    .Attrs({"relu: int", "precision: int"})
    .SetKernelFn(PD_KERNEL(p3d_gather_gemm_op))
    .SetInferShapeFn(PD_INFER_SHAPE(GgInferShape))
    .SetInferDtypeFn(PD_INFER_DTYPE(GgInferDtype));

std::vector<paddle::Tensor> p3d_rows_to_h16_op(const paddle::Tensor &rows, const paddle::Tensor &num, const paddle::Tensor &status) {
  P3D_CHECK_GPU(rows);
  const int64_t cap = rows.shape()[0];
  const int C = static_cast<int>(rows.shape()[1]);
  auto out = paddle::empty({cap, 2 * C}, paddle::DataType::FLOAT16, paddle::GPUPlace());
  P3D_CALL(p3d_rows_convert_h16(rows.data<float>(), 1, num.data<int>(), cap, C, out.data(), const_cast<int *>(status.data<int>()),
                                rows.stream()));
  return {out};
}
std::vector<std::vector<int64_t>> ToH16InferShape(std::vector<int64_t> r, std::vector<int64_t> n, std::vector<int64_t> s) {
  return {{r[0], 2 * r[1]}};
}
std::vector<paddle::DataType> ToH16InferDtype(paddle::DataType r, paddle::DataType n, paddle::DataType s) {
  return {paddle::DataType::FLOAT16};
}
PD_BUILD_OP(p3d_rows_to_h16)
    .Inputs({"ROWS", "NUM", "STATUS"})
    .Outputs({"OUT"})
    .SetKernelFn(PD_KERNEL(p3d_rows_to_h16_op))
    .SetInferShapeFn(PD_INFER_SHAPE(ToH16InferShape))
    .SetInferDtypeFn(PD_INFER_DTYPE(ToH16InferDtype));

std::vector<paddle::Tensor> p3d_sparse_conv_f16_op(const paddle::Tensor &in, const paddle::Tensor &nbr, const paddle::Tensor &num,
                                                   const paddle::Tensor &weight, const paddle::Tensor &scale,
                                                   const paddle::Tensor &shift, const paddle::Tensor &residual,
                                                   const paddle::Tensor &status, const int cin, const int cout, const int relu,
                                                   const int want_f32, const int max_splits) {
  P3D_CHECK_GPU(in);
  const int64_t cap = nbr.shape()[0];
  const int K = static_cast<int>(nbr.shape()[1]);
  auto out = want_f32 ? paddle::empty({cap, cout}, paddle::DataType::FLOAT32, paddle::GPUPlace())
                      : paddle::empty({cap, 2 * cout}, paddle::DataType::FLOAT16, paddle::GPUPlace());
  const size_t ws_bytes = p3d_sparse_conv_f16_workspace_bytes(cap, cout, max_splits);
  auto ws = paddle::full({static_cast<int64_t>(ws_bytes ? ws_bytes : 16)}, 0, paddle::DataType::UINT8, paddle::GPUPlace());
  const void *res = residual.numel() > 1 ? residual.data() : nullptr;
  P3D_CALL(p3d_sparse_conv_f16(in.data(), nbr.data<int>(), num.data<int>(), cap, K, cin, cout, weight.data(), scale.data<float>(),
                               shift.data<float>(), res, relu, want_f32 ? out.data<float>() : nullptr,
                               want_f32 ? nullptr : out.data(), ws_bytes ? ws.data<uint8_t>() : nullptr, ws_bytes, max_splits,
                               const_cast<int *>(status.data<int>()), in.stream()));
  return {out};
}
std::vector<std::vector<int64_t>> ScF16InferShape(std::vector<int64_t> in, std::vector<int64_t> nbr, std::vector<int64_t> num,
                                                  std::vector<int64_t> w, std::vector<int64_t> sc, std::vector<int64_t> sh,
                                                  std::vector<int64_t> res, std::vector<int64_t> st, const int &cin,
                                                  const int &cout, const int &relu, const int &want_f32, const int &max_splits) {
  return {{nbr[0], want_f32 ? static_cast<int64_t>(cout) : static_cast<int64_t>(2 * cout)}};
}
std::vector<paddle::DataType> ScF16InferDtype(paddle::DataType in, paddle::DataType nbr, paddle::DataType num, paddle::DataType w,
                                              paddle::DataType sc, paddle::DataType sh, paddle::DataType res, paddle::DataType st) {
  return {in};
}
PD_BUILD_OP(p3d_sparse_conv_f16)
    .Inputs({"IN", "NBR", "NUM", "WEIGHT", "SCALE", "SHIFT", "RESIDUAL", "STATUS"})
    .Outputs({"OUT"})
    .Attrs({"cin: int", "cout: int", "relu: int", "want_f32: int", "max_splits: int"})
    .SetKernelFn(PD_KERNEL(p3d_sparse_conv_f16_op))
    .SetInferShapeFn(PD_INFER_SHAPE(ScF16InferShape))
    .SetInferDtypeFn(PD_INFER_DTYPE(ScF16InferDtype));

std::vector<paddle::Tensor> p3d_sparse_conv_wm_op(const paddle::Tensor &in, const paddle::Tensor &nbr, const paddle::Tensor &num,
                                                  const paddle::Tensor &weight, const paddle::Tensor &scale,
                                                  const paddle::Tensor &shift, const paddle::Tensor &residual,
                                                  const paddle::Tensor &status, const int cin, const int cout, const int relu,
                                                  const int want_f32) {
  P3D_CHECK_GPU(in);
  const int64_t cap = nbr.shape()[0];
  const int K = static_cast<int>(nbr.shape()[1]);
  auto out = want_f32 ? paddle::empty({cap, cout}, paddle::DataType::FLOAT32, paddle::GPUPlace())
                      : paddle::empty({cap, 2 * cout}, paddle::DataType::FLOAT16, paddle::GPUPlace());
  const size_t ws_bytes = p3d_sparse_conv_wm_workspace_bytes(cap, cout);
  auto ws = paddle::full({static_cast<int64_t>(ws_bytes ? ws_bytes : 16)}, 0, paddle::DataType::UINT8, paddle::GPUPlace());
  const void *res = residual.numel() > 1 ? residual.data() : nullptr;
  P3D_CALL(p3d_sparse_conv_wm(in.data(), nbr.data<int>(), num.data<int>(), cap, K, cin, cout, weight.data(), scale.data<float>(),
                              shift.data<float>(), res, relu, want_f32 ? out.data<float>() : nullptr,
                              want_f32 ? nullptr : out.data(), ws.data<uint8_t>(), ws_bytes,
                              const_cast<int *>(status.data<int>()), in.stream()));
  return {out};
}
std::vector<std::vector<int64_t>> ScWmInferShape(std::vector<int64_t> in, std::vector<int64_t> nbr, std::vector<int64_t> num,
                                                 std::vector<int64_t> w, std::vector<int64_t> sc, std::vector<int64_t> sh,
                                                 std::vector<int64_t> res, std::vector<int64_t> st, const int &cin,
                                                 const int &cout, const int &relu, const int &want_f32) {
  return {{nbr[0], want_f32 ? static_cast<int64_t>(cout) : static_cast<int64_t>(2 * cout)}};
}
PD_BUILD_OP(p3d_sparse_conv_wm)
    .Inputs({"IN", "NBR", "NUM", "WEIGHT", "SCALE", "SHIFT", "RESIDUAL", "STATUS"})
    .Outputs({"OUT"})
    .Attrs({"cin: int", "cout: int", "relu: int", "want_f32: int"})
    .SetKernelFn(PD_KERNEL(p3d_sparse_conv_wm_op))
    .SetInferShapeFn(PD_INFER_SHAPE(ScWmInferShape))
    .SetInferDtypeFn(PD_INFER_DTYPE(ScF16InferDtype));

std::vector<paddle::Tensor> p3d_dense_conv2d_f16_op(const paddle::Tensor &image, const paddle::Tensor &weight,
                                                    const paddle::Tensor &scale, const paddle::Tensor &shift,
                                                    const paddle::Tensor &status, const std::vector<int> &bhwc, const int cout,
                                                    const int n_tile, const int kernel, const int stride, const int pad,
                                                    const int up, const int relu, const int out_channels, const int out_c0) {
  P3D_CHECK_GPU(image);
  const int B = bhwc[0], H = bhwc[1], W = bhwc[2], Cin = bhwc[3];
  const int oH = up > 1 ? H * up : (H + 2 * pad - kernel) / stride + 1, oW = up > 1 ? W * up : (W + 2 * pad - kernel) / stride + 1;
  auto out = paddle::empty({static_cast<int64_t>(B) * oH * oW, 2 * out_channels}, paddle::DataType::FLOAT16, paddle::GPUPlace());
  const int k = up > 1 ? up : kernel, s = up > 1 ? up : stride;
  P3D_CALL(p3d_dense_conv2d_f16(image.data(), B, H, W, Cin, weight.data(), cout, n_tile, k, k, s, up > 1 ? 0 : pad, up,
                                scale.data<float>(), shift.data<float>(), relu, out.data(), out_channels, out_c0, nullptr, 0, 0,
                                const_cast<int *>(status.data<int>()), image.stream()));
  return {out};
}
std::vector<std::vector<int64_t>> DcF16InferShape(std::vector<int64_t> im, std::vector<int64_t> w, std::vector<int64_t> sc,
                                                  std::vector<int64_t> sh, std::vector<int64_t> st, const std::vector<int> &bhwc,
                                                  const int &cout, const int &n_tile, const int &kernel, const int &stride,
                                                  const int &pad, const int &up, const int &relu, const int &out_channels,
                                                  const int &out_c0) {
  const int64_t oH = up > 1 ? bhwc[1] * up : (bhwc[1] + 2 * pad - kernel) / stride + 1;
  const int64_t oW = up > 1 ? bhwc[2] * up : (bhwc[2] + 2 * pad - kernel) / stride + 1;
  return {{bhwc[0] * oH * oW, 2 * static_cast<int64_t>(out_channels)}};
}
std::vector<paddle::DataType> DcF16InferDtype(paddle::DataType im, paddle::DataType w, paddle::DataType sc, paddle::DataType sh,
                                              paddle::DataType st) {
  return {paddle::DataType::FLOAT16};
}
PD_BUILD_OP(p3d_dense_conv2d_f16)
    .Inputs({"IMAGE", "WEIGHT", "SCALE", "SHIFT", "STATUS"})
    .Outputs({"OUT"})
    .Attrs({"bhwc: std::vector<int>", "cout: int", "n_tile: int", "kernel: int", "stride: int", "pad: int", "up: int",
            "relu: int", "out_channels: int", "out_c0: int"})
    .SetKernelFn(PD_KERNEL(p3d_dense_conv2d_f16_op))
    .SetInferShapeFn(PD_INFER_SHAPE(DcF16InferShape))
    .SetInferDtypeFn(PD_INFER_DTYPE(DcF16InferDtype));

std::vector<paddle::Tensor> p3d_bev_pool_prepare_op(const paddle::Tensor &coor, const std::vector<float> &lower,
                                                    const std::vector<float> &interval, const std::vector<int> &grid_size) {
  P3D_CHECK_GPU(coor);
  const auto sh = coor.shape();
  const int B = sh[0], N = sh[1], D = sh[2], H = sh[3], W = sh[4];
  const int64_t n = static_cast<int64_t>(B) * N * D * H * W;
  std::vector<paddle::Tensor> out;
  for (int i = 0; i < 5; ++i) out.push_back(paddle::empty({n}, paddle::DataType::INT32, paddle::GPUPlace()));
  out.push_back(paddle::empty({2}, paddle::DataType::INT32, paddle::GPUPlace()));
  const size_t ws_bytes = p3d_bev_pool_prepare_workspace_bytes(n);
  auto ws = workspace(ws_bytes);
  P3D_CALL(p3d_bev_pool_prepare(coor.data<float>(), B, N, D, H, W, lower.data(), interval.data(), grid_size.data(),
                                out[0].data<int>(), out[1].data<int>(), out[2].data<int>(), out[3].data<int>(), out[4].data<int>(),
                                out[5].data<int>(), ws.data<uint8_t>(), ws_bytes, coor.stream()));
  return out;
}
std::vector<std::vector<int64_t>> PrepInferShape(std::vector<int64_t> c, const std::vector<float> &lower,
                                                 const std::vector<float> &interval, const std::vector<int> &grid_size) {
  const int64_t n = c[0] * c[1] * c[2] * c[3] * c[4];
  return {{n}, {n}, {n}, {n}, {n}, {2}};
}
std::vector<paddle::DataType> PrepInferDtype(paddle::DataType c) {
  return {paddle::DataType::INT32, paddle::DataType::INT32, paddle::DataType::INT32, paddle::DataType::INT32,
          paddle::DataType::INT32, paddle::DataType::INT32};
}
PD_BUILD_OP(p3d_bev_pool_prepare)
    .Inputs({"COOR"})
    .Outputs({"RANKS_BEV", "RANKS_DEPTH", "RANKS_FEAT", "INTERVAL_STARTS", "INTERVAL_LENGTHS", "COUNTS"})
    .Attrs({"grid_lower_bound: std::vector<float>", "grid_interval: std::vector<float>", "grid_size: std::vector<int>"})
    .SetKernelFn(PD_KERNEL(p3d_bev_pool_prepare_op))
    .SetInferShapeFn(PD_INFER_SHAPE(PrepInferShape))
    .SetInferDtypeFn(PD_INFER_DTYPE(PrepInferDtype));
```

Baseline: 381.6.

## Add stream-K split of dense conv K-loop with slab reduction to fix wave quantization

Adds a stream-K schedule to the warp-specialized dense f16 conv kernel: the K-dimension units (taps × channel groups) of all output tiles are evenly split across a grid of at most one CTA per SM. Partial tiles write fp32 slabs to a workspace, and an atomic ticket picks the last CTA to sum the slabs before running the normal epilogue. A cost model picks stream-K only when it beats the tail-wave cost of the plain tile schedule, and it also drives the m_tiles choice. The Python path supplies a zeroed workspace, while the Paddle op passes none and keeps the old schedule. This trades global-memory slab traffic and cross-CTA fences for better SM balance on tile counts that do not divide evenly into waves.

```diff
diff --git a/include/p3d_b200.h b/include/p3d_b200.h
--- a/include/p3d_b200.h
+++ b/include/p3d_b200.h
@@ -173,6 +173,8 @@
                           p3d_stream_t stream);
 int p3d_pixel_h16_to_nchw(const void *in_h16, int B, int C, int H, int W, float *out, p3d_stream_t stream);
 size_t p3d_dense_conv2d_f16_packed_weight_bytes(int taps, int Cin, int Cout, int n_tile);
+size_t p3d_dense_conv2d_f16_workspace_bytes(int B, int H, int W, int Cout, int n_tile, int kh, int kw, int stride, int pad,
+                                            int up);
 int p3d_dense_conv2d_f16_pack_weights(const float *weight_tci, int taps, int Cin, int n_tile, void *packed,
                                       int32_t *status_dev, p3d_stream_t stream);
 size_t p3d_bev_pool_prepare_workspace_bytes(int64_t num_points);
@@ -189,8 +191,8 @@
                           int planes, float *out_nchw, p3d_stream_t stream);
 int p3d_dense_conv2d_f16(const void *in_h16, int B, int H, int W, int Cin, const void *packed_weight, int Cout, int n_tile,
                          int kh, int kw, int stride, int pad, int up, const float *scale, const float *shift, int relu,
-                         void *out_h16, int out_C, int out_c0, float *out_nchw, int mode, int m_tiles,
-                         int32_t *status_dev, p3d_stream_t stream);
+                         void *out_h16, int out_C, int out_c0, float *out_nchw, int mode, int m_tiles, void *workspace,
+                         size_t workspace_bytes, int32_t *status_dev, p3d_stream_t stream);
 
 int p3d_pillar_feature_net(const float *voxels, const int32_t *num_points_per_voxel, const int32_t *coors,
                            const int32_t *num_voxels_dev, int64_t n_cap, int max_points, int num_point_dim,
diff --git a/paddle3d_b200/_lib.py b/paddle3d_b200/_lib.py
--- a/paddle3d_b200/_lib.py
+++ b/paddle3d_b200/_lib.py
@@ -81,7 +81,8 @@
     "p3d_head_out_conv_f16": (_int, [_vp, _int, _int, _int, _int, _int, _int, _vp, _vp, _vp, _vp, _vp, _int, _vp, _vp]),
     "p3d_grouped_head_conv_f16": (_int, [_vp, _int, _int, _int, _int, _int, _int, _vp, _vp, _vp, _vp, _int, _vp, _vp, _vp]),
     "p3d_dense_conv2d_f16": (_int, [_vp, _int, _int, _int, _int, _vp, _int, _int, _int, _int, _int, _int, _int, _vp, _vp,
-                                    _int, _vp, _int, _int, _vp, _int, _int, _vp, _vp]),
+                                    _int, _vp, _int, _int, _vp, _int, _int, _vp, _sz, _vp, _vp]),
+    "p3d_dense_conv2d_f16_workspace_bytes": (_sz, [_int] * 10),
     "p3d_dense_conv2d_split": (_int, [_vp, _int, _int, _int, _int, _vp, _int, _int, _int, _int, _int, _int, _int, _vp, _vp,
                                       _int, _vp, _int, _int, _vp, _vp]),
     "p3d_sparse_conv_gather_gemm_tf32x3_ws": (_int, [_vp, _vp, _vp, _i64, _int, _int, _int, _vp, _vp, _vp, _vp, _int, _vp,
diff --git a/paddle3d_b200/csrc/dense_conv_f16.cu b/paddle3d_b200/csrc/dense_conv_f16.cu
--- a/paddle3d_b200/csrc/dense_conv_f16.cu
+++ b/paddle3d_b200/csrc/dense_conv_f16.cu
@@ -35,6 +35,9 @@
   const int32_t *grp_plane0, *grp_cnt;
   int base_offset_mode;
   int w_bytes;
+  int sk;
+  int32_t *tickets;
+  float *slabs;
 };
 
 template <int N, int MT, bool HALO, int PITCH, bool WS = false>
@@ -107,6 +110,7 @@
   kTrStageFree = kTrEpi + 2,
   kTrAEmpty = kTrStageFree + 2, kTrBEmpty,
   kTrEwWait, kTrEwBusy,
+  kTrSlabWr, kTrSlabSum,
   kTrFields
 };
 #ifdef P3D_DENSE_TRACE
@@ -158,21 +162,133 @@
   return it;
 }
 
+struct Sched {
+  long long w_first, w_step, n_items;
+  int total, u0, u1;
+  int U;
+  __device__ __forceinline__ void units(long long idx, int &ua, int &ub) const {
+    if (total == 0) {
+      ua = 0;
+      ub = U;
+      return;
+    }
+    const int s = static_cast<int>(w_first + idx) * U;
+    ua = u0 > s ? u0 - s : 0;
+    ub = u1 < s + U ? u1 - s : U;
+  }
+  __device__ __forceinline__ int cta_of(int x) const {
+    return static_cast<int>(((x + 1ll) * gridDim.x - 1) / total);
+  }
+  __device__ __forceinline__ int slot(int cta, int t) const {
+    return static_cast<int>(static_cast<long long>(cta) * total / gridDim.x) / U == t ? 0 : 1;
+  }
+};
+template <bool WS>
+__device__ __forceinline__ Sched make_sched(const Params &p, long long n_total, int U) {
+  Sched s;
+  s.U = U;
+  s.total = s.u0 = s.u1 = 0;
+  if (p.sk) {
+    s.total = static_cast<int>(n_total) * U;
+    s.u0 = static_cast<int>(static_cast<long long>(blockIdx.x) * s.total / gridDim.x);
+    s.u1 = static_cast<int>(static_cast<long long>(blockIdx.x + 1) * s.total / gridDim.x);
+    s.w_first = s.u0 / U;
+    s.w_step = 1;
+    s.n_items = s.u1 > s.u0 ? (s.u1 - 1) / U - s.w_first + 1 : 0;
+  } else if (WS) {
+    s.w_first = (static_cast<long long>(blockIdx.x) * n_total) / gridDim.x;
+    s.w_step = 1;
+    s.n_items = (static_cast<long long>(blockIdx.x + 1) * n_total) / gridDim.x - s.w_first;
+  } else {
+    s.w_first = blockIdx.x;
+    s.w_step = gridDim.x;
+    s.n_items = s.w_first < n_total ? (n_total - s.w_first + s.w_step - 1) / s.w_step : 0;
+  }
+  return s;
+}
+
+__device__ __forceinline__ void epi_bar() { asm volatile("bar.sync 1, 96;" ::: "memory"); }
+__device__ __forceinline__ void fence_gpu() { asm volatile("fence.acq_rel.gpu;" ::: "memory"); }
+
 template <int N, int MT>
-__device__ __forceinline__ void epilogue_warps(const Params &p, const float *stg, unsigned long long *staged,
-                                               unsigned long long *freed, long long n_items, long long w_first,
-                                               long long w_step, int th, int et) {
+__device__ __forceinline__ void epilogue_warps(const Params &p, const Sched &sc, float *stg, unsigned long long *staged,
+                                               unsigned long long *freed, int *s_last, int th, int et) {
   constexpr int SP = N + 8, ROWS = MT * 64;
+  constexpr int SLAB = 2 * ROWS * N;
   const int ew = et >> 5, lane = et & 31;
+  auto stg4 = [&](int e) { return reinterpret_cast<float4 *>(stg + (e / (N / 4)) * SP) + e % (N / 4); };
   bool ovf = false;
   Trace tr;
-  for (long long idx = 0; idx < n_items; ++idx) {
-    const Item im = decode<false>(w_first + idx * w_step, p, th);
+  for (long long idx = 0; idx < sc.n_items; ++idx) {
+    const long long t = sc.w_first + idx * sc.w_step;
+    const Item im = decode<false>(t, p, th);
     const int g_cnt = p.grouped ? __ldg(p.grp_cnt + im.nt) : 0, g_p0 = p.grouped ? __ldg(p.grp_plane0 + im.nt) : 0;
     const int dy = p.up > 1 ? im.tap0 / p.up : 0, dx = p.up > 1 ? im.tap0 % p.up : 0;
+    int ua, ub;
+    sc.units(idx, ua, ub);
+    const bool partial = ub - ua < sc.U;
+    if (partial) {
+      long long t0 = tr.now();
+      mbar_wait(smem_u32(staged + 0), static_cast<uint32_t>(idx & 1));
+      mbar_wait(smem_u32(staged + 1), static_cast<uint32_t>(idx & 1));
+      tr.add(kTrEwWait, t0);
+      t0 = tr.now();
+      float *mine = p.slabs + (static_cast<size_t>(blockIdx.x) * 2 + (idx == 0 ? 0 : 1)) * SLAB;
+#pragma unroll 1
+      for (int e = et; e < SLAB / 4; e += kEpiThreads)
+        __stcg(reinterpret_cast<float4 *>(mine) + e, *stg4(e));
+      fence_gpu();
+      epi_bar();
+      const int cf = sc.cta_of(static_cast<int>(t) * sc.U), cl = sc.cta_of(static_cast<int>(t) * sc.U + sc.U - 1);
+      const int pieces = cl - cf + 1, piece = static_cast<int>(blockIdx.x) - cf;
+      if (et == 0) {
+        int old;
+        asm volatile("atom.acq_rel.gpu.global.add.s32 %0, [%1], 1;" : "=r"(old) : "l"(p.tickets + t) : "memory");
+        const int last = old == pieces - 1;
+        if (last) p.tickets[t] = 0;
+        *s_last = last;
+      }
+      epi_bar();
+      const bool last = *s_last != 0;
+      tr.add(kTrSlabWr, t0);
+      if (!last) {
+        mbar_arrive(smem_u32(freed + 0));
+        mbar_arrive(smem_u32(freed + 1));
+        continue;
+      }
+      t0 = tr.now();
+      fence_gpu();
+      constexpr int kSumBatch = 6;
+      for (int sp = piece == 0 ? 1 : 0; sp < pieces; ++sp) {
+        const float4 *src = reinterpret_cast<const float4 *>(
+            p.slabs + (static_cast<size_t>(cf + sp) * 2 + (sp == 0 ? sc.slot(cf, static_cast<int>(t)) : 0)) * SLAB);
+        for (int e0 = et; e0 < SLAB / 4; e0 += kSumBatch * kEpiThreads) {
+          float4 x[kSumBatch];
+#pragma unroll
+          for (int k = 0; k < kSumBatch; ++k)
+            if (e0 + k * kEpiThreads < SLAB / 4) x[k] = __ldcg(src + e0 + k * kEpiThreads);
+#pragma unroll
+          for (int k = 0; k < kSumBatch; ++k) {
+            const int e = e0 + k * kEpiThreads;
+            if (e >= SLAB / 4) break;
+            float4 *o = stg4(e);
+            if (sp > 0) {
+              const float4 a = *o;
+              x[k].x += a.x;
+              x[k].y += a.y;
+              x[k].z += a.z;
+              x[k].w += a.w;
+            }
+            *o = x[k];
+          }
+        }
+      }
+      epi_bar();
+      tr.add(kTrSlabSum, t0);
+    }
     for (int c = 0; c < 2; ++c) {
       long long t0 = tr.now();
-      mbar_wait(smem_u32(staged + c), static_cast<uint32_t>(idx & 1));
+      if (!partial) mbar_wait(smem_u32(staged + c), static_cast<uint32_t>(idx & 1));
       tr.add(kTrEwWait, t0);
       t0 = tr.now();
       const float *st = stg + c * ROWS * SP;
@@ -246,15 +362,17 @@
   asm volatile("griddepcontrol.wait;" ::: "memory");
   const int up2 = p.up * p.up;
   const long long n_total = static_cast<long long>(p.B) * p.tiles_y * p.tiles_x * p.n_ntiles * (p.up > 1 ? up2 : 1);
-  if (static_cast<long long>(blockIdx.x) >= n_total) return;
-  const long long w_first = WS ? (static_cast<long long>(blockIdx.x) * n_total) / gridDim.x : blockIdx.x;
-  const long long n_work = WS ? (static_cast<long long>(blockIdx.x + 1) * n_total) / gridDim.x : n_total;
-  const long long w_step = WS ? 1 : gridDim.x;
-  const long long n_items = (n_work - w_first + w_step - 1) / w_step;
+  const int G = p.Cin / 32;
+  const int taps_item = p.up > 1 ? 1 : p.taps;
+  const int units_item = HALO ? G : taps_item * G;
+  const Sched sc = make_sched<WS>(p, n_total, units_item);
+  if (sc.n_items == 0) return;
+  const long long n_items = sc.n_items;
 
   extern __shared__ __align__(1024) uint8_t smem_raw[];
   uint8_t *smem = reinterpret_cast<uint8_t *>((reinterpret_cast<uintptr_t>(smem_raw) + 1023) & ~uintptr_t(1023));
   __shared__ __align__(8) unsigned long long s_bar[2 * kMaxA + 2 * kMaxB + 6];
+  __shared__ int s_last;
   constexpr int kAF = 0, kAE = kMaxA, kBF = 2 * kMaxA, kBE = 2 * kMaxA + kMaxB, kWF = 2 * kMaxA + 2 * kMaxB, kWE = kWF + 1;
   constexpr int kSS = kWE + 1, kSF = kSS + 2;
 
@@ -280,15 +398,12 @@
   const uint32_t a_ring = smem_u32(smem);
   const uint32_t b_ring = a_ring + C::NA * C::A_BYTES;
   float *const stg = reinterpret_cast<float *>(smem + C::NA * C::A_BYTES + C::NB * C::B_BYTES);
-  const int G = p.Cin / 32;
-  const int taps_item = p.up > 1 ? 1 : p.taps;
-  const int units_item = HALO ? G : taps_item * G;
-  auto item_w = [&](long long idx) { return w_first + idx * w_step; };
+  auto item_w = [&](long long idx) { return sc.w_first + idx * sc.w_step; };
 
   if (wg == 0) {
     asm volatile("setmaxnreg.dec.sync.aligned.u32 %0;" ::"n"(C::P_REGS));
     if (tid >= 32) {
-      if (C::STAGE) epilogue_warps<N, MT>(p, stg, s_bar + kSS, s_bar + kSF, n_items, w_first, w_step, TH, tid - 32);
+      if (C::STAGE) epilogue_warps<N, MT>(p, sc, stg, s_bar + kSS, s_bar + kSF, &s_last, TH, tid - 32);
       return;
     }
     if (tid != 0) return;
@@ -311,34 +426,34 @@
         ++img;
         cur_nt = im.nt;
       }
-      int dy = 0, dx = 0;
-      for (int tu = 0; tu < (HALO ? 1 : taps_item); ++tu) {
+      int ua, ub;
+      sc.units(idx, ua, ub);
+      for (int u = ua; u < ub; ++u) {
+        const int g = HALO ? u : u % G, tu = HALO ? 0 : u / G;
         const int tap = p.up > 1 ? im.tap0 : tu;
-        for (int g = 0; g < G; ++g) {
-          const uint32_t abar = smem_u32(&s_bar[kAF + a_slot]), a_dst = a_ring + a_slot * C::A_BYTES;
-          const long long t0 = tr.now();
-          mbar_wait(smem_u32(&s_bar[kAE + a_slot]), a_ph ^ 1u);
-          tr.add(kTrAEmpty, t0);
-          mbar_arrive_expect_tx(abar, static_cast<uint32_t>(C::A_ROWS * 128));
-          if (HALO) {
-            tma_tile4d(a_dst, &in_map, (cg0 + g) * 64, im.tx0 - 1, im.ty0 - 1, im.b, abar);
-          } else {
-            const int x = im.tx0 * p.stride - p.pad + dx, y = im.ty0 * p.stride - p.pad + dy;
-            tma_tile4d(a_dst, &in_map, (cg0 + g) * 64, x, y, im.b, abar);
-          }
-          if (++a_slot == C::NA) a_slot = 0, a_ph ^= 1u;
-          for (int t = 0; t < (WS ? 0 : C::SPU); ++t) {
-            const uint32_t bbar = smem_u32(&s_bar[kBF + b_slot]);
-            const long long t1 = tr.now();
-            mbar_wait(smem_u32(&s_bar[kBE + b_slot]), b_ph ^ 1u);
-            tr.add(kTrBEmpty, t1);
-            mbar_arrive_expect_tx(bbar, static_cast<uint32_t>(C::B_BYTES));
-            bulk_g2s(b_ring + b_slot * C::B_BYTES, w_tile + (static_cast<size_t>(HALO ? t : tap) * (p.Cin / 16) + 2 * g) * C::B_BLK,
-                     static_cast<uint32_t>(C::B_BYTES), bbar);
-            if (++b_slot == C::NB) b_slot = 0, b_ph ^= 1u;
-          }
-        }
-        if (++dx == p.kw) dx = 0, ++dy;
+        const int dy = p.up > 1 ? 0 : tu / p.kw, dx = p.up > 1 ? 0 : tu % p.kw;
+        const uint32_t abar = smem_u32(&s_bar[kAF + a_slot]), a_dst = a_ring + a_slot * C::A_BYTES;
+        const long long t0 = tr.now();
+        mbar_wait(smem_u32(&s_bar[kAE + a_slot]), a_ph ^ 1u);
+        tr.add(kTrAEmpty, t0);
+        mbar_arrive_expect_tx(abar, static_cast<uint32_t>(C::A_ROWS * 128));
+        if (HALO) {
+          tma_tile4d(a_dst, &in_map, (cg0 + g) * 64, im.tx0 - 1, im.ty0 - 1, im.b, abar);
+        } else {
+          const int x = im.tx0 * p.stride - p.pad + dx, y = im.ty0 * p.stride - p.pad + dy;
+          tma_tile4d(a_dst, &in_map, (cg0 + g) * 64, x, y, im.b, abar);
+        }
+        if (++a_slot == C::NA) a_slot = 0, a_ph ^= 1u;
+        for (int t = 0; t < (WS ? 0 : C::SPU); ++t) {
+          const uint32_t bbar = smem_u32(&s_bar[kBF + b_slot]);
+          const long long t1 = tr.now();
+          mbar_wait(smem_u32(&s_bar[kBE + b_slot]), b_ph ^ 1u);
+          tr.add(kTrBEmpty, t1);
+          mbar_arrive_expect_tx(bbar, static_cast<uint32_t>(C::B_BYTES));
+          bulk_g2s(b_ring + b_slot * C::B_BYTES, w_tile + (static_cast<size_t>(HALO ? t : tap) * (p.Cin / 16) + 2 * g) * C::B_BLK,
+                   static_cast<uint32_t>(C::B_BYTES), bbar);
+          if (++b_slot == C::NB) b_slot = 0, b_ph ^= 1u;
+        }
       }
     }
     tr.flush(0);
@@ -370,7 +485,9 @@
     uint32_t prev_b = 0;
     int prev_a = -1;
     bool pending = false;
-    for (int ua = 0; ua < units_item; ++ua) {
+    int ua, ub;
+    sc.units(idx, ua, ub);
+    for (int u = ua; u < ub; ++u) {
       long long t0 = tr.now();
       mbar_wait(smem_u32(&s_bar[kAF + a_slot]), a_ph);
       tr.add(kTrAFull, t0);
@@ -379,7 +496,7 @@
         t0 = tr.now();
         if (!WS) mbar_wait(smem_u32(&s_bar[kBF + b_slot]), b_ph);
         tr.add(kTrBFull, t0);
-        const uint32_t b_base = WS ? b_ring + static_cast<uint32_t>((t * (p.Cin / 16) + 2 * ua) * C::B_BLK)
+        const uint32_t b_base = WS ? b_ring + static_cast<uint32_t>((t * (p.Cin / 16) + 2 * u) * C::B_BLK)
                                    : b_ring + b_slot * C::B_BYTES;
         wg_fence();
 #pragma unroll
@@ -564,17 +681,16 @@
 }
 
 template <int N, int MT, bool HALO, int PITCH, bool WS = false>
-int launch(const CUtensorMap &map, const Params &p, cudaStream_t st) {
+int launch(const CUtensorMap &map, const Params &p, long long grid, cudaStream_t st) {
   using C = Cfg<N, MT, HALO, PITCH, WS>;
   const size_t smem = static_cast<size_t>(C::NA) * C::A_BYTES +
                       (WS ? static_cast<size_t>(p.w_bytes) : static_cast<size_t>(C::NB) * C::B_BYTES) + C::STG_BYTES + 1024;
   if (smem > static_cast<size_t>(227 - 6) * 1024) return P3D_ERR_UNSUPPORTED;
+  if (WS && p.sk) return P3D_ERR_UNSUPPORTED;
   auto kern = dense_conv_f16_kernel<N, MT, HALO, PITCH, WS>;
   P3D_CUDA_CHECK(cudaFuncSetAttribute(kern, cudaFuncAttributeMaxDynamicSharedMemorySize, static_cast<int>(smem)));
-  const long long work = static_cast<long long>(p.B) * p.tiles_y * p.tiles_x * p.n_ntiles * (p.up > 1 ? p.up * p.up : 1);
   cudaLaunchConfig_t cfg = {};
-  const long long sms = num_sms();
-  cfg.gridDim = dim3(static_cast<unsigned int>(work < sms ? work : sms));
+  cfg.gridDim = dim3(static_cast<unsigned int>(grid));
   cfg.blockDim = dim3(kDenseThreads);
   cfg.dynamicSmemBytes = smem;
   cfg.stream = st;
@@ -772,10 +888,30 @@
   return align_up(tiles * taps * Cin * static_cast<size_t>(n_tile) * 4);
 }
 
+static size_t dense_ws_tickets(int B, int oH, int oW, int Cout, int n_tile, int up) {
+  const size_t items = static_cast<size_t>(B) * ((oH + dcf::kTH - 1) / dcf::kTH) * ((oW + dcf::kTW - 1) / dcf::kTW) *
+                       ((Cout + n_tile - 1) / n_tile) * (up > 1 ? up * up : 1);
+  return align_up(items * sizeof(int32_t));
+}
+static size_t dense_ws_slabs(int n_tile) {
+  return 2 * static_cast<size_t>(num_sms()) * 128 * n_tile * (n_tile <= 64 ? 2 : 1) * sizeof(float);
+}
+
+extern "C" size_t p3d_dense_conv2d_f16_workspace_bytes(int B, int H, int W, int Cout, int n_tile, int kh, int kw, int stride,
+                                                       int pad, int up) {
+  if (B < 1 || H < 1 || W < 1 || Cout < 1 || (n_tile != 64 && n_tile != 128) || up < 1 || kh < 1 || kw < 1 || stride < 1 ||
+      pad < 0)
+    return 0;
+  const int oH = up > 1 ? H : (H + 2 * pad - kh) / stride + 1, oW = up > 1 ? W : (W + 2 * pad - kw) / stride + 1;
+  if (oH < 1 || oW < 1) return 0;
+  return dense_ws_tickets(B, oH, oW, Cout, n_tile, up) + dense_ws_slabs(n_tile);
+}
+
 static int dense_conv_f16(const void *in_h16, int B, int H, int W, int Cin, const void *packed_weight, int Cout, int n_tile,
                           int kh, int kw, int stride, int pad, int up, const float *scale, const float *shift, int relu,
-                          void *out_h16, int out_C, int out_c0, float *out_nchw, int mode, int m_tiles, int32_t *status_dev,
-                          p3d_stream_t stream, int groups, int in_C, const int32_t *grp_plane0, const int32_t *grp_cnt) {
+                          void *out_h16, int out_C, int out_c0, float *out_nchw, int mode, int m_tiles, void *workspace,
+                          size_t workspace_bytes, int32_t *status_dev, p3d_stream_t stream, int groups, int in_C,
+                          const int32_t *grp_plane0, const int32_t *grp_cnt) {
   if (!in_h16 || !packed_weight || (!out_h16 && !out_nchw) || B < 1 || H < 1 || W < 1 || Cout < 1) return P3D_ERR_INVALID_ARG;
   if (Cin < 32 || Cin % 32 || (n_tile != 64 && n_tile != 128 && !(groups && n_tile == 16))) return P3D_ERR_UNSUPPORTED;
   if (up < 1 || (up > 1 && (kh != up || kw != up || stride != up || pad != 0))) return P3D_ERR_UNSUPPORTED;
@@ -823,12 +959,36 @@
   if (env_mode >= 0) mode = env_mode;
   if (env_mt >= 0) m_tiles = env_mt;
   const bool halo = (mode == 0 || mode == 2) && up == 1 && kh == 3 && kw == 3 && stride == 1 && pad == 1;
+  constexpr long long kSkFixSteps = 64;
+  const long long sms = num_sms();
+  const long long U = (halo ? 1 : (up > 1 ? 1 : p.taps)) * (Cin / 32), spu = halo ? 9 : 1;
+  const char *env_sk = getenv("P3D_DENSE_STREAMK");
+  const int force_sk = env_sk ? atoi(env_sk) : -1;
+  if (workspace && !groups) {
+    if (reinterpret_cast<uintptr_t>(workspace) & 15) return P3D_ERR_INVALID_ARG;
+    if (workspace_bytes < p3d_dense_conv2d_f16_workspace_bytes(B, H, W, Cout, n_tile, kh, kw, stride, pad, up))
+      return P3D_ERR_WORKSPACE;
+  }
+  struct Plan {
+    long long cost, grid;
+    bool sk;
+  };
+  auto plan = [&](long long items, int m) {
+    Plan r{(items + sms - 1) / sms * U * spu * m, items < sms ? items : sms, false};
+    const long long total = items * U;
+    if (!workspace || groups || force_sk == 0 || total >= (1ll << 31)) return r;
+    const long long u_min = (U + 1) / 3 > 1 ? (U + 1) / 3 : 1;
+    const long long g = total / u_min < sms ? total / u_min : sms;
+    const long long cost = (total + g - 1) / g * spu * m + kSkFixSteps;
+    if (force_sk == 1 || (items >= sms && cost < r.cost)) r = Plan{cost, g, true};
+    return r;
+  };
   int mt = m_tiles;
   if (mt != 1 && mt != 2) {
-    const long long tx = (p.oW + dcf::kTW - 1) / dcf::kTW, sms = num_sms();
+    const long long tx = (p.oW + dcf::kTW - 1) / dcf::kTW;
     const long long per_row = static_cast<long long>(B) * tx * p.n_ntiles * (up > 1 ? up * up : 1);
     const long long items1 = per_row * ((p.oH + dcf::kTH - 1) / dcf::kTH), items2 = per_row * ((p.oH + 2 * dcf::kTH - 1) / (2 * dcf::kTH));
-    mt = (n_tile <= 64 && 2 * ((items2 + sms - 1) / sms) <= (items1 + sms - 1) / sms) ? 2 : 1;
+    mt = (n_tile <= 64 && plan(items2, 2).cost <= plan(items1, 1).cost) ? 2 : 1;
   }
   static const int env_ws = getenv("P3D_DENSE_WS") ? atoi(getenv("P3D_DENSE_WS")) : 0;
   p.w_bytes = p.taps * (Cin / 16) * 64 * n_tile;
@@ -844,17 +1004,24 @@
   if (mt == 2) pitch = 10;
   p.tiles_x = (p.oW + dcf::kTW - 1) / dcf::kTW;
   p.tiles_y = (p.oH + dcf::kTH * mt - 1) / (dcf::kTH * mt);
+  const long long items = static_cast<long long>(B) * p.tiles_y * p.tiles_x * p.n_ntiles * (up > 1 ? up * up : 1);
+  const Plan pl = ws ? Plan{0, items < sms ? items : sms, false} : plan(items, mt);
+  const long long grid = pl.grid;
+  p.sk = pl.sk ? 1 : 0;
+  p.tickets = pl.sk ? static_cast<int32_t *>(workspace) : nullptr;
+  p.slabs = pl.sk ? reinterpret_cast<float *>(static_cast<char *>(workspace) + dense_ws_tickets(B, p.oH, p.oW, Cout, n_tile, up))
+                  : nullptr;
   CUtensorMap map;
   const int bx = halo ? pitch : dcf::kTW, by = halo ? dcf::kTH * mt + 2 : dcf::kTH * mt;
   const int rc = dcf::make_image_map(in_h16, B, H, W, p.in_C, p.stride, bx, by, &map);
   if (rc != P3D_OK) return rc;
   cudaStream_t st = static_cast<cudaStream_t>(stream);
-  if (ws) return dcf::launch<64, 1, true, 10, true>(map, p, st);
-#define P3D_DCF(NT, M)                                                                          \
-  if (n_tile == NT && mt == M) {                                                                \
-    if (!halo) return dcf::launch<NT, M, false, 10>(map, p, st);                                \
-    if (M == 1 && pitch == 16) return dcf::launch<NT, 1, true, 16>(map, p, st);                 \
-    return dcf::launch<NT, M, true, 10>(map, p, st);                                            \
+  if (ws) return dcf::launch<64, 1, true, 10, true>(map, p, grid, st);
+#define P3D_DCF(NT, M)                                                                 \
+  if (n_tile == NT && mt == M) {                                                       \
+    if (!halo) return dcf::launch<NT, M, false, 10>(map, p, grid, st);                 \
+    if (M == 1 && pitch == 16) return dcf::launch<NT, 1, true, 16>(map, p, grid, st);  \
+    return dcf::launch<NT, M, true, 10>(map, p, grid, st);                             \
   }
   P3D_DCF(16, 1)
   P3D_DCF(16, 2)
@@ -868,9 +1035,11 @@
 extern "C" int p3d_dense_conv2d_f16(const void *in_h16, int B, int H, int W, int Cin, const void *packed_weight, int Cout,
                                     int n_tile, int kh, int kw, int stride, int pad, int up, const float *scale,
                                     const float *shift, int relu, void *out_h16, int out_C, int out_c0, float *out_nchw,
-                                    int mode, int m_tiles, int32_t *status_dev, p3d_stream_t stream) {
+                                    int mode, int m_tiles, void *workspace, size_t workspace_bytes, int32_t *status_dev,
+                                    p3d_stream_t stream) {
   return dense_conv_f16(in_h16, B, H, W, Cin, packed_weight, Cout, n_tile, kh, kw, stride, pad, up, scale, shift, relu, out_h16,
-                        out_C, out_c0, out_nchw, mode, m_tiles, status_dev, stream, 0, 0, nullptr, nullptr);
+                        out_C, out_c0, out_nchw, mode, m_tiles, workspace, workspace_bytes, status_dev, stream, 0, 0, nullptr,
+                        nullptr);
 }
 
 extern "C" int p3d_grouped_head_conv_f16(const void *in_h16, int B, int H, int W, int in_C, int Cin, int groups,
@@ -879,7 +1048,7 @@
                                          p3d_stream_t stream) {
   if (!plane0_dev || !cnt_dev || groups < 1 || groups * Cin > in_C || in_C % 32 || planes < 1) return P3D_ERR_INVALID_ARG;
   return dense_conv_f16(in_h16, B, H, W, Cin, packed_weight, planes, 16, 3, 3, 1, 1, 1, nullptr, bias, 0, nullptr, 32, 0, out_nchw,
-                        0, 0, status_dev, stream, groups, in_C, plane0_dev, cnt_dev);
+                        0, 0, nullptr, 0, status_dev, stream, groups, in_C, plane0_dev, cnt_dev);
 }
 
 extern "C" int p3d_head_out_conv_f16(const void *in_h16, int B, int H, int W, int in_C, int Cin, int groups,
diff --git a/paddle3d_b200/ops/dense_conv.py b/paddle3d_b200/ops/dense_conv.py
--- a/paddle3d_b200/ops/dense_conv.py
+++ b/paddle3d_b200/ops/dense_conv.py
@@ -1,7 +1,7 @@
 import torch
 
 from .._lib import check, lib
-from .._mem import ptr, require_cuda, stream
+from .._mem import ptr, require_cuda, stream, workspace
 
 
 def n_tile_for(cout):
@@ -150,7 +150,10 @@
     if out_h16 is None and not want_nchw:
         out_h16 = torch.empty((b * oh * ow, 2 * oc), dtype=torch.float16, device=dev)
     out_nchw = torch.empty((b, cout, oh, ow), dtype=torch.float32, device=dev) if want_nchw else None
-    check(lib().p3d_dense_conv2d_f16(ptr(x_h16), b, h, w, cin, ptr(packed), int(cout), int(n_tile), kh, kw, st, pd, int(up),
-                                     ptr(scale), ptr(shift), int(relu), ptr(out_h16), oc, int(out_c0), ptr(out_nchw),
-                                     int(mode), int(m_tiles), ptr(_status(dev)), stream(dev)), "dense_conv2d_f16")
+    L = lib()
+    wsb = L.p3d_dense_conv2d_f16_workspace_bytes(b, h, w, int(cout), int(n_tile), kh, kw, st, pd, int(up))
+    ws = workspace(wsb, dev, "dense_streamk", zero=True) if wsb else None
+    check(L.p3d_dense_conv2d_f16(ptr(x_h16), b, h, w, cin, ptr(packed), int(cout), int(n_tile), kh, kw, st, pd, int(up),
+                                 ptr(scale), ptr(shift), int(relu), ptr(out_h16), oc, int(out_c0), ptr(out_nchw),
+                                 int(mode), int(m_tiles), ptr(ws), wsb, ptr(_status(dev)), stream(dev)), "dense_conv2d_f16")
     return out_h16, out_nchw, (b, oh, ow)
diff --git a/paddle_ext/p3d_paddle_ops.cc b/paddle_ext/p3d_paddle_ops.cc
--- a/paddle_ext/p3d_paddle_ops.cc
+++ b/paddle_ext/p3d_paddle_ops.cc
@@ -491,7 +491,7 @@
   const int k = up > 1 ? up : kernel, s = up > 1 ? up : stride;
   P3D_CALL(p3d_dense_conv2d_f16(image.data(), B, H, W, Cin, weight.data(), cout, n_tile, k, k, s, up > 1 ? 0 : pad, up,
                                 scale.data<float>(), shift.data<float>(), relu, out.data(), out_channels, out_c0, nullptr, 0, 0,
-                                const_cast<int *>(status.data<int>()), image.stream()));
+                                nullptr, 0, const_cast<int *>(status.data<int>()), image.stream()));
   return {out};
 }
 std::vector<std::vector<int64_t>> DcF16InferShape(std::vector<int64_t> im, std::vector<int64_t> w, std::vector<int64_t> sc,
```

Result: no change. 379.6, median of 6 (-0.5%).
